# speedinghzl/DSRG

Hardware: AMD Instinct MI355X
Metric: images/sec DSRG train step (VGG16 321x321, 21-class) (higher is better)
Workload: dtype bf16 backbone (fp32 master weights) + f32/f64 supervision path

## Files before the change

dsrg_amd/csrc/conv_igemm.hip:

```cpp
#include "common.h"
#include "igemm_plan.h"
#include <algorithm>
#include <cstring>
#include <vector>

namespace dsrg {
namespace {
typedef __attribute__((ext_vector_type(8))) __bf16 bf16x8;
typedef __attribute__((ext_vector_type(2))) __bf16 bf16x2;
typedef __attribute__((ext_vector_type(2))) float f32x2;
typedef __attribute__((ext_vector_type(16))) float f32x16;
typedef __attribute__((ext_vector_type(4))) float f32x4;
typedef __attribute__((address_space(3))) void lds_void;

constexpr int kOutRow = 128 * 2 + 16;
constexpr int kOutWave = 64 * kOutRow;
constexpr uint32_t kOob = 0x80000000u;
constexpr int kRowTab = 8 * kOutWave;
constexpr int kRowTabBytes = kBM * 4;

template <int BK, int NST> struct ICfg {
    static constexpr int ROW = BK * 2;
    static constexpr int CPR = ROW / 16;
    static constexpr int RPI = 1024 / ROW;
    static constexpr int IPW = 256 / RPI / 8;
    static constexpr int STAGE = (kBM + kBN) * ROW;
    static constexpr int KS = BK / 16;
    static constexpr int SPC = 64 / BK;
    static constexpr int AHEAD = NST - 1;
    static_assert(NST * STAGE <= kRowTab, "the row table sits behind the stages");
    static constexpr size_t LDS = (size_t)kRowTab + kRowTabBytes;
    __device__ static constexpr int swz(int r) { return BK == 64 ? (r >> 1) & 7 : (r >> 2) & 3; }
};

struct IgemmClass {
    uint32_t rect;
    int q0;
};
struct IgemmGroup {
    const uint16_t *x;
    const uint16_t *w;
    const float *bias;
    uint16_t *y;
    const uint16_t *mask;
    float *colsum;
    const uint16_t *res;
    int dil, ncls;
    IgemmClass cls[kMaxClasses];
};
struct IgemmArgs {
    IgemmGroup g[4];
    int ngroups, B, H, W, Cin, Cout, taps, relu, M, tiles_m, tiles_n, tiles_per_group;
    int stagger;
    uint32_t drop_thresh;
    float drop_scale;
    uint32_t seed_lo, seed_hi;
    float out_scale;
    int xcd_mix;
    int row_tiles, rows_per_tile, bands;
    int skip_taps;
    int xrow;
    int cpp;
    int out_f32;
    int cls_tiles;
};

__device__ __forceinline__ uint32_t fmix32(uint32_t h) {
    h ^= h >> 16; h *= 0x85EBCA6Bu; h ^= h >> 13; h *= 0xC2B2AE35u; h ^= h >> 16;
    return h;
}
__device__ __forceinline__ uint32_t dropout_bytes(uint32_t e4, uint32_t seed_lo, uint32_t seed_hi) {
    return fmix32(fmix32(e4 ^ seed_lo) + seed_hi);
}

__device__ __forceinline__ uint32_t pack2(float lo, float hi) {
    f32x2 v = {lo, hi};
    bf16x2 b = __builtin_convertvector(v, bf16x2);
    return *reinterpret_cast<uint32_t *>(&b);
}

template <int N> __device__ __forceinline__ void wait_vm_barrier() {
    asm volatile("s_waitcnt vmcnt(%0)\n\ts_barrier" ::"n"(N) : "memory");
}

constexpr int kAhead = 3;
struct IgemmFrag {
    uint32_t choff[2];
    __device__ __forceinline__ explicit IgemmFrag(int lane) {
        using C = ICfg<64, 2>;
        const int l15 = lane & 15, g4 = lane >> 4;
#pragma unroll
        for (int sl = 0; sl < 2; sl++) choff[sl] = (uint32_t)l15 * C::ROW + (uint32_t)(((sl * 4 + g4) ^ C::swz(l15)) << 4);
    }
};
template <class LateIssue>
__device__ __forceinline__ void igemm_mma_step(const unsigned char *P, const unsigned char *Wt, const IgemmFrag &fr, f32x4 (&acc)[8][4],
                                               const bool late, LateIssue &&late_issue) {
    using C = ICfg<64, 2>;
    constexpr int RING = kAhead + 1;
    bf16x8 bq[2][4], ar[RING];
    auto read_w = [&](int u) { return *reinterpret_cast<const bf16x8 *>(Wt + (u & 7) * (16 * C::ROW) + fr.choff[u >> 3]); };
#pragma unroll
    for (int j = 0; j < 4; j++) bq[0][j] = *reinterpret_cast<const bf16x8 *>(P + j * (16 * C::ROW) + fr.choff[0]);
#pragma unroll
    for (int u = 0; u < kAhead; u++) ar[u] = read_w(u);
#pragma unroll
    for (int u = 0; u < 16; u++) {
        if (u + kAhead < 16) ar[(u + kAhead) % RING] = read_w(u + kAhead);
        if (u < 4) bq[1][u] = *reinterpret_cast<const bf16x8 *>(P + u * (16 * C::ROW) + fr.choff[1]);
        __builtin_amdgcn_sched_barrier(0);
#pragma unroll
        for (int j = 0; j < 4; j++)
            acc[u & 7][j] = __builtin_amdgcn_mfma_f32_16x16x32_bf16(ar[u % RING], bq[u >> 3][j], acc[u & 7][j], 0, 0, 0);
        __builtin_amdgcn_sched_barrier(0);
        if (u == 3 && late) late_issue();
    }
}

__device__ __forceinline__ void conv_igemm_body(const IgemmArgs &a, const int bid, const int nblk) {
    using C = ICfg<64, 2>;
    extern __shared__ __attribute__((aligned(16))) unsigned char ig_lds[];
    const int tid = threadIdx.x, lane = tid & 63;
    const int wv = __builtin_amdgcn_readfirstlane(tid >> 6);
    const int l15 = lane & 15, g4 = lane >> 4;
    const int wn = wv >> 2, wm = wv & 3;

    int grp, tm, tn;
    if (a.xcd_mix) {
        const int id = bid, xcd = id & 7, k = id >> 3;
        const int cm = (a.tiles_m - xcd + 7) >> 3, per_group = cm * a.tiles_n;
        if (cm <= 0 || k >= per_group * a.ngroups) return;
        grp = k / per_group;
        const int r = k - grp * per_group, tml = r / a.tiles_n;
        tn = r - tml * a.tiles_n;
        tm = xcd + 8 * tml;
    } else {
        const int total = nblk, id = bid;
        const int q = total >> 3, r = total & 7, xcd = id & 7, k = id >> 3;
        int t = (xcd < r ? xcd * (q + 1) : r * (q + 1) + (xcd - r) * q) + k;
        grp = t / a.tiles_per_group;
        t -= grp * a.tiles_per_group;
        tm = t / a.tiles_n;
        tn = t - tm * a.tiles_n;
    }
    int m0 = tm * kBM, mvalid;
    if (a.row_tiles) {
        const int bimg = tm / a.bands, band = tm - bimg * a.bands, row0 = band * a.rows_per_tile;
        m0 = (bimg * a.H + row0) * a.W;
        mvalid = min(a.rows_per_tile, a.H - row0) * a.W;
    } else {
        mvalid = min(kBM, a.M - m0);
    }
    const int n0 = tn * kBN;
    const IgemmGroup &G = a.g[grp];
    const int taps = a.taps, Cin = a.Cin, W = a.W, H = a.H;
    const int ktot = taps * Cin;
    volatile int32_t *rowpix = reinterpret_cast<volatile int32_t *>(ig_lds + kRowTab);
    const bool cls = a.cls_tiles != 0;
    if (cls) {
        if (tid < kBM) {
            const int q = m0 + tid;
            int m = -1;
            if (q < a.M) {
                uint32_t rect = G.cls[0].rect;
                int q0 = G.cls[0].q0;
#pragma unroll
                for (int k = 1; k < kMaxClasses; k++)
                    if (k < G.ncls && q >= G.cls[k].q0) { rect = G.cls[k].rect; q0 = G.cls[k].q0; }
                const int cy0 = (int)(rect & 255u), ch = (int)((rect >> 8) & 255u), cx0 = (int)((rect >> 16) & 255u), cw = (int)(rect >> 24);
                const int qq = q - q0, area = ch * cw, b = qq / area, rem = qq - b * area, yy = rem / cw, xx = rem - yy * cw;
                m = (b * H + cy0 + yy) * W + cx0 + xx;
            }
            rowpix[tid] = m;
        }
        __syncthreads();
    }
    auto row_pixel = [&](int r) -> int { return cls ? rowpix[r] : (r < mvalid ? m0 + r : -1); };

    const int xrow = a.xrow;
    const rsrc_t rx = make_rsrc(G.x, (size_t)a.M * xrow);
    const rsrc_t rw = make_rsrc(G.w, (size_t)a.Cout * ktot * 2);

    uint32_t pbase[C::IPW], pvalid[C::IPW], wbase[C::IPW];
#pragma unroll
    for (int i = 0; i < C::IPW; i++) {
        const int r = wv * 32 + i * C::RPI + lane / C::CPR;
        const int c = (lane % C::CPR) ^ C::swz(r);
        const int m = row_pixel(r);
        const bool in = m >= 0;
        const int mm = in ? m : 0;
        const int hw = H * W;
        const int b = mm / hw, rem = mm - b * hw, y = rem / W, x = rem - y * W;
        uint32_t valid = 0;
        if (in) {
            if (taps == 9) {
#pragma unroll
                for (int tap = 0; tap < 9; tap++) {
                    const int yy = y + (tap / 3 - 1) * G.dil, xx = x + (tap % 3 - 1) * G.dil;
                    if (yy >= 0 && yy < H && xx >= 0 && xx < W) valid |= 1u << tap;
                }
            } else {
                valid = 1u;
            }
        }
        pbase[i] = (uint32_t)mm * (uint32_t)xrow + (uint32_t)c * 16u;
        pvalid[i] = valid;
        wbase[i] = (uint32_t)(n0 + r) * (uint32_t)(ktot * 2) + (uint32_t)c * 16u;
    }

    uint32_t tapmask = taps == 9 ? 0x1ffu : 1u;
    if (a.skip_taps && taps == 9 && G.dil >= 3) {
        uint32_t v = 0;
#pragma unroll
        for (int i = 0; i < C::IPW; i++) v |= pvalid[i];
#pragma unroll
        for (int o = 32; o; o >>= 1) v |= (uint32_t)__shfl_xor((int)v, o);
        volatile uint32_t *red = reinterpret_cast<volatile uint32_t *>(ig_lds);
        if (lane == 0) red[wv] = v;
        __syncthreads();
        v = 0;
#pragma unroll
        for (int k = 0; k < 8; k++) v |= red[k];
        __syncthreads();
        tapmask = (uint32_t)__builtin_amdgcn_readfirstlane((int)v);
    }
    unsigned long long taplist = 0;
    int nlive = 0;
#pragma unroll
    for (int tp = 0; tp < 9; tp++)
        if ((tapmask >> tp) & 1u) { taplist |= (unsigned long long)tp << (4 * nlive); nlive++; }
    const int nsteps = (Cin >> 6) * nlive * C::SPC;

    int it_cc = 0, it_tap = 0, it_h = 0;
    auto issue = [&](int stage, int) {
        const int tap = (int)((taplist >> (4 * it_tap)) & 15u);
        const int cc = it_cc, h = it_h;
        const uint32_t s_real = (uint32_t)((cc * taps + tap) * C::SPC + h);
        if (++it_h == C::SPC) { it_h = 0; if (++it_tap == nlive) { it_tap = 0; it_cc++; } }
        int dy = 0, dx = 0;
        if (taps == 9) { dy = tap / 3 - 1; dx = tap - (tap / 3) * 3 - 1; }
        const int xc = a.cpp ? (int)((0x610u >> (2 * (cc / a.cpp))) & 3u) * a.cpp + cc % a.cpp : cc;
        const int toff = (dy * G.dil * W + dx * G.dil) * xrow + xc * 128 + h * C::ROW;
        unsigned char *P = ig_lds + stage * C::STAGE + wv * (32 * C::ROW);
        unsigned char *Wt = P + kBM * C::ROW;
#pragma unroll
        for (int i = 0; i < C::IPW; i++) {
            const uint32_t vo = ((pvalid[i] >> tap) & 1u) ? pbase[i] + (uint32_t)toff : kOob;
            __builtin_amdgcn_raw_ptr_buffer_load_lds(rx, (lds_void *)(P + i * (C::RPI * C::ROW)), 16, vo, 0, 0, 0);
        }
#pragma unroll
        for (int i = 0; i < C::IPW; i++)
            __builtin_amdgcn_raw_ptr_buffer_load_lds(rw, (lds_void *)(Wt + i * (C::RPI * C::ROW)), 16, wbase[i], s_real * C::ROW, 0, 0);
    };

    f32x4 acc[8][4];
#pragma unroll
    for (int i = 0; i < 8; i++)
#pragma unroll
        for (int j = 0; j < 4; j++)
#pragma unroll
            for (int r = 0; r < 4; r++) acc[i][j][r] = 0.0f;

    const IgemmFrag fr(lane);
    const bool active = n0 + wn * 128 < a.Cout;
    const bool late = a.stagger && wv >= 4 && active;
    if (nsteps > 0) issue(0, 0);
    if (!active) {
        for (int s = 0; s < nsteps; s++) {
            wait_vm_barrier<0>();
            if (s + 1 < nsteps) issue((s & 1) ^ 1, s + 1);
        }
    } else {
        for (int s = 0; s < nsteps; s++) {
            const int stage = s & 1;
            wait_vm_barrier<0>();
            const bool more = s + 1 < nsteps;
            if (more && !late) issue(stage ^ 1, s + 1);
            igemm_mma_step(ig_lds + stage * C::STAGE + wm * (64 * C::ROW), ig_lds + stage * C::STAGE + kBM * C::ROW + wn * (128 * C::ROW), fr, acc,
                           more && late, [&]() { issue(stage ^ 1, s + 1); });
        }
    }
    __syncthreads();
    if (!active) return;

    unsigned char *O = ig_lds + wv * kOutWave;
    const int nw = n0 + wn * 128;
    if (a.out_f32) {
        float *y32 = reinterpret_cast<float *>(G.y);
        const float floor32 = a.relu ? 0.0f : -__builtin_inff();
#pragma unroll
        for (int j = 0; j < 4; j++) {
            const int m = row_pixel(wm * 64 + j * 16 + l15);
#pragma unroll
            for (int i = 0; i < 8; i++) {
                const int n = nw + i * 16 + g4 * 4;
                float4 b4 = make_float4(0.f, 0.f, 0.f, 0.f);
                if (G.bias) b4 = *reinterpret_cast<const float4 *>(G.bias + n);
                const float4 v = make_float4(fmaxf(acc[i][j][0] + b4.x, floor32), fmaxf(acc[i][j][1] + b4.y, floor32),
                                             fmaxf(acc[i][j][2] + b4.z, floor32), fmaxf(acc[i][j][3] + b4.w, floor32));
                if (m >= 0) *reinterpret_cast<float4 *>(y32 + (size_t)m * a.Cout + n) = v;
            }
        }
        return;
    }
    const rsrc_t rb = make_rsrc(G.bias, G.bias ? (size_t)a.Cout * 4 : 0);
    const float floor_ = (a.relu && !G.res) ? 0.0f : -__builtin_inff();
    const uint32_t seed_g = a.seed_lo + (uint32_t)grp * 0x9E3779B9u;
    float bias_r[8][4];
#pragma unroll
    for (int i = 0; i < 8; i++)
#pragma unroll
        for (int e = 0; e < 4; e++) bias_r[i][e] = ld_f32(rb, (uint32_t)(nw + i * 16 + g4 * 4 + e) * 4u);
#pragma unroll
    for (int i = 0; i < 8; i++) {
        const int nl = i * 16 + g4 * 4;
#pragma unroll
        for (int j = 0; j < 4; j++) {
            float v0 = acc[i][j][0] + bias_r[i][0], v1 = acc[i][j][1] + bias_r[i][1];
            float v2 = acc[i][j][2] + bias_r[i][2], v3 = acc[i][j][3] + bias_r[i][3];
            v0 = fmaxf(v0, floor_) * a.out_scale; v1 = fmaxf(v1, floor_) * a.out_scale;
            v2 = fmaxf(v2, floor_) * a.out_scale; v3 = fmaxf(v3, floor_) * a.out_scale;
            if (a.drop_thresh) {
                const uint32_t m = cls ? (uint32_t)rowpix[wm * 64 + j * 16 + l15] : (uint32_t)(m0 + wm * 64 + j * 16 + l15);
                const uint32_t h = dropout_bytes((m * (uint32_t)a.Cout + (uint32_t)(nw + nl)) >> 2, seed_g, a.seed_hi);
                v0 = (h & 0xffu) >= a.drop_thresh ? v0 * a.drop_scale : 0.0f;
                v1 = ((h >> 8) & 0xffu) >= a.drop_thresh ? v1 * a.drop_scale : 0.0f;
                v2 = ((h >> 16) & 0xffu) >= a.drop_thresh ? v2 * a.drop_scale : 0.0f;
                v3 = (h >> 24) >= a.drop_thresh ? v3 * a.drop_scale : 0.0f;
            }
            *reinterpret_cast<uint2 *>(O + (j * 16 + l15) * kOutRow + nl * 2) = make_uint2(pack2(v0, v1), pack2(v2, v3));
        }
    }
    const bool chv = nw + (lane & 15) * 8 < a.Cout;
    if (G.res) {
        const float floor2 = a.relu ? 0.0f : -__builtin_inff();
#pragma unroll
        for (int h = 0; h < 2; h++) {
            uint4 rs[8], mk8[8];
#pragma unroll
            for (int it = 0; it < 8; it++) {
                const int m = row_pixel(wm * 64 + (h * 8 + it) * 4 + (lane >> 4));
                const size_t at = (size_t)m * a.Cout + nw + (lane & 15) * 8;
                rs[it] = (m >= 0 && chv) ? *reinterpret_cast<const uint4 *>(G.res + at) : make_uint4(0, 0, 0, 0);
                mk8[it] = !G.mask ? make_uint4(0x3f803f80u, 0x3f803f80u, 0x3f803f80u, 0x3f803f80u)
                                  : ((m >= 0 && chv) ? *reinterpret_cast<const uint4 *>(G.mask + at) : make_uint4(0, 0, 0, 0));
            }
#pragma unroll
            for (int it = 0; it < 8; it++) {
                const int p = (h * 8 + it) * 4 + (lane >> 4), ch = lane & 15;
                const int m = row_pixel(wm * 64 + p);
                const uint4 v = *reinterpret_cast<const uint4 *>(O + p * kOutRow + ch * 16);
                uint32_t w4[4] = {v.x, v.y, v.z, v.w};
                const uint32_t r4[4] = {rs[it].x, rs[it].y, rs[it].z, rs[it].w};
                const uint32_t y4[4] = {mk8[it].x, mk8[it].y, mk8[it].z, mk8[it].w};
#pragma unroll
                for (int e = 0; e < 4; e++) {
                    const float lo = fmaxf(__uint_as_float(w4[e] << 16) + __uint_as_float(r4[e] << 16), floor2);
                    const float hi = fmaxf(__uint_as_float(w4[e] & 0xffff0000u) + __uint_as_float(r4[e] & 0xffff0000u), floor2);
                    const uint32_t klo = (int16_t)(y4[e] & 0xffffu) > 0 ? 0x0000ffffu : 0u;
                    const uint32_t khi = (int32_t)y4[e] >= 0x10000 ? 0xffff0000u : 0u;
                    w4[e] = pack2(lo, hi) & (klo | khi);
                }
                if (m >= 0 && chv) *reinterpret_cast<uint4 *>(G.y + (size_t)m * a.Cout + nw + ch * 8) = make_uint4(w4[0], w4[1], w4[2], w4[3]);
            }
        }
        return;
    }
    if (!G.mask && !G.colsum) {
#pragma unroll 4
        for (int it = 0; it < 16; it++) {
            const int p = it * 4 + (lane >> 4), ch = lane & 15;
            const int m = row_pixel(wm * 64 + p);
            const uint4 v = *reinterpret_cast<const uint4 *>(O + p * kOutRow + ch * 16);
            if (m >= 0 && chv) *reinterpret_cast<uint4 *>(G.y + (size_t)m * a.Cout + nw + ch * 8) = v;
        }
        return;
    }
    uint4 mk[16];
    if (G.mask) {
#pragma unroll
        for (int it = 0; it < 16; it++) {
            const int m = row_pixel(wm * 64 + it * 4 + (lane >> 4));
            mk[it] = (m >= 0 && chv) ? *reinterpret_cast<const uint4 *>(G.mask + (size_t)m * a.Cout + nw + (lane & 15) * 8) : make_uint4(0, 0, 0, 0);
        }
    } else {
#pragma unroll
        for (int it = 0; it < 16; it++) mk[it] = make_uint4(0x3f803f80u, 0x3f803f80u, 0x3f803f80u, 0x3f803f80u);
    }
    float cs[8] = {0, 0, 0, 0, 0, 0, 0, 0};
#pragma unroll
    for (int it = 0; it < 16; it++) {
        const int p = it * 4 + (lane >> 4), ch = lane & 15;
        const int m = row_pixel(wm * 64 + p);
        const uint4 v = *reinterpret_cast<const uint4 *>(O + p * kOutRow + ch * 16);
        uint32_t w4[4] = {v.x, v.y, v.z, v.w};
        const uint32_t y4[4] = {mk[it].x, mk[it].y, mk[it].z, mk[it].w};
#pragma unroll
        for (int e = 0; e < 4; e++) {
            const uint32_t lo = (int16_t)(y4[e] & 0xffffu) > 0 ? 0x0000ffffu : 0u;
            const uint32_t hi = (int32_t)y4[e] >= 0x10000 ? 0xffff0000u : 0u;
            w4[e] &= lo | hi;
            cs[2 * e] += __uint_as_float(w4[e] << 16);
            cs[2 * e + 1] += __uint_as_float(w4[e] & 0xffff0000u);
        }
        if (m >= 0 && chv) *reinterpret_cast<uint4 *>(G.y + (size_t)m * a.Cout + nw + ch * 8) = make_uint4(w4[0], w4[1], w4[2], w4[3]);
    }
    if (G.colsum) {
#pragma unroll
        for (int e = 0; e < 8; e++) {
            cs[e] += __shfl_xor(cs[e], 16);
            cs[e] += __shfl_xor(cs[e], 32);
        }
        float *slab = reinterpret_cast<float *>(O);
        if (lane < 16) {
            *reinterpret_cast<float4 *>(slab + lane * 8) = make_float4(cs[0], cs[1], cs[2], cs[3]);
            *reinterpret_cast<float4 *>(slab + lane * 8 + 4) = make_float4(cs[4], cs[5], cs[6], cs[7]);
        }
        __syncthreads();
        if (wm == 0) {
            const float *s0 = reinterpret_cast<const float *>(ig_lds + (wn * 4 + 0) * kOutWave);
            const float *s1 = reinterpret_cast<const float *>(ig_lds + (wn * 4 + 1) * kOutWave);
            const float *s2 = reinterpret_cast<const float *>(ig_lds + (wn * 4 + 2) * kOutWave);
            const float *s3 = reinterpret_cast<const float *>(ig_lds + (wn * 4 + 3) * kOutWave);
            float *dst = G.colsum + (size_t)tm * a.Cout + nw;
            dst[lane] = (s0[lane] + s1[lane]) + (s2[lane] + s3[lane]);
            if (nw + lane + 64 < a.Cout) dst[lane + 64] = (s0[lane + 64] + s1[lane + 64]) + (s2[lane + 64] + s3[lane + 64]);
        }
    }
}


__global__ __launch_bounds__(512, 2) void conv_igemm_kernel_64x2(IgemmArgs a) { conv_igemm_body(a, (int)blockIdx.x, (int)gridDim.x); }

struct IgemmSkArgs {
    IgemmArgs base;
    float *ws;
    uint32_t *flags;
    int units, tiles_total;
};
constexpr int kSkParts = 4;
using f32x4v = decltype(__builtin_amdgcn_raw_buffer_load_b128(rsrc_t(), 0, 0, 0));

__global__ __launch_bounds__(512, 2) void conv_igemm_sk_kernel(IgemmSkArgs k) {
    using C = ICfg<64, 2>;
    const IgemmArgs &a = k.base;
    extern __shared__ __attribute__((aligned(16))) unsigned char ig_lds[];
    const int tid = threadIdx.x, lane = tid & 63;
    const int wv = __builtin_amdgcn_readfirstlane(tid >> 6);
    const int l15 = lane & 15, g4 = lane >> 4;
    const int wn = wv >> 2, wm = wv & 3;
    int unit;
    {
        const int total = (int)gridDim.x, id = (int)blockIdx.x;
        const int q = total >> 3, r = total & 7, xcd = id & 7, kk = id >> 3;
        unit = (xcd < r ? xcd * (q + 1) : r * (q + 1) + (xcd - r) * q) + kk;
    }
    const int taps = a.taps, Cin = a.Cin, W = a.W, H = a.H;
    const int ktot = taps * Cin;
    const int nsteps = (Cin >> 6) * taps;
    const long long total_steps = (long long)k.tiles_total * nsteps;
    auto unit_start = [&](int u) { return (long long)u * total_steps / k.units; };
    const long long g1 = unit_start(unit + 1);
    const IgemmFrag fr(lane);
    const rsrc_t rws = make_rsrc(k.ws, (size_t)k.units * 32 * 512 * 16);
    const float floor_ = a.relu ? 0.0f : -__builtin_inff();

    for (long long g = unit_start(unit); g < g1;) {
        const int tile = (int)(g / nsteps);
        const int sb = (int)(g - (long long)tile * nsteps);
        const int se = (int)min((long long)nsteps, sb + (g1 - g));
        int t = tile;
        const int grp = t / a.tiles_per_group;
        t -= grp * a.tiles_per_group;
        const int tm = t / a.tiles_n, tn = t - tm * a.tiles_n;
        const int m0 = tm * kBM, n0 = tn * kBN;
        const IgemmGroup G = a.g[grp];
        const rsrc_t rx = make_rsrc(G.x, (size_t)a.M * Cin * 2);
        const rsrc_t rw = make_rsrc(G.w, (size_t)a.Cout * ktot * 2);
        const bool active = n0 + wn * 128 < a.Cout;

        uint32_t pbase0, wbase0, pvalid01 = 0, pvalid23 = 0;
        {
            const int r0 = wv * 32 + lane / C::CPR;
            const int c0 = (lane % C::CPR) ^ C::swz(r0);
            pbase0 = (uint32_t)(m0 + r0) * (uint32_t)(Cin * 2) + (uint32_t)c0 * 16u;
            wbase0 = (uint32_t)(n0 + r0) * (uint32_t)(ktot * 2) + (uint32_t)c0 * 16u;
#pragma unroll
            for (int i = 0; i < C::IPW; i++) {
                const int m = m0 + r0 + i * C::RPI;
                uint32_t valid = 0;
                if (m < a.M) {
                    const int hw = H * W;
                    const int bimg = m / hw, rem = m - bimg * hw, y = rem / W, x = rem - y * W;
                    if (taps == 9) {
#pragma unroll
                        for (int tap = 0; tap < 9; tap++) {
                            const int yy = y + (tap / 3 - 1) * G.dil, xx = x + (tap % 3 - 1) * G.dil;
                            if (yy >= 0 && yy < H && xx >= 0 && xx < W) valid |= 1u << tap;
                        }
                    } else {
                        valid = 1u;
                    }
                }
                if (i < 2) pvalid01 |= valid << (16 * i); else pvalid23 |= valid << (16 * (i - 2));
            }
        }
        auto issue = [&](int stage, int s) {
            const int cc = s / taps, tap = s - cc * taps;
            int dy = 0, dx = 0;
            if (taps == 9) { dy = tap / 3 - 1; dx = tap - (tap / 3) * 3 - 1; }
            const int toff = (dy * G.dil * W + dx * G.dil) * Cin * 2 + cc * 128;
            unsigned char *P = ig_lds + stage * C::STAGE + wv * (32 * C::ROW);
            unsigned char *Wt = P + kBM * C::ROW;
#pragma unroll
            for (int i = 0; i < C::IPW; i++) {
                const uint32_t bits = (i < 2 ? pvalid01 : pvalid23) >> (16 * (i & 1) + tap);
                const uint32_t off = ((pbase0 + (uint32_t)(i * C::RPI * Cin * 2)) ^ ((i & 1) ? 64u : 0u)) + (uint32_t)toff;
                __builtin_amdgcn_raw_ptr_buffer_load_lds(rx, (lds_void *)(P + i * (C::RPI * C::ROW)), 16, (bits & 1u) ? off : kOob, 0, 0, 0);
            }
#pragma unroll
            for (int i = 0; i < C::IPW; i++)
                __builtin_amdgcn_raw_ptr_buffer_load_lds(rw, (lds_void *)(Wt + i * (C::RPI * C::ROW)), 16, (i & 1) ? wbase0 ^ 64u : wbase0,
                                                         (uint32_t)s * C::ROW + (uint32_t)(i * C::RPI * ktot * 2), 0, 0);
        };

        f32x4 acc[8][4];
#pragma unroll
        for (int i = 0; i < 8; i++)
#pragma unroll
            for (int j = 0; j < 4; j++)
#pragma unroll
                for (int r = 0; r < 4; r++) acc[i][j][r] = 0.0f;

        issue(0, sb);
        if (!active) {
            for (int s = sb; s < se; s++) {
                wait_vm_barrier<0>();
                if (s + 1 < se) issue(((s - sb) & 1) ^ 1, s + 1);
            }
        } else {
            for (int s = sb; s < se; s++) {
                const int stage = (s - sb) & 1;
                wait_vm_barrier<0>();
                const bool more = s + 1 < se, late = wv >= 4;
                if (more && !late) issue(stage ^ 1, s + 1);
                igemm_mma_step(ig_lds + stage * C::STAGE + wm * (64 * C::ROW), ig_lds + stage * C::STAGE + kBM * C::ROW + wn * (128 * C::ROW), fr, acc,
                               more && late, [&]() { issue(stage ^ 1, s + 1); });
            }
        }
        __syncthreads();

        if (sb != 0) {
            if (active) {
#pragma unroll
                for (int i = 0; i < 8; i++)
#pragma unroll
                    for (int j = 0; j < 4; j++) {
                        f32x4v v = {__float_as_uint(acc[i][j][0]), __float_as_uint(acc[i][j][1]), __float_as_uint(acc[i][j][2]), __float_as_uint(acc[i][j][3])};
                        __builtin_amdgcn_raw_buffer_store_b128(v, rws, (uint32_t)((i * 4 + j) * 512 + tid) * 16u,
                                                               (uint32_t)unit * (32u * 512u * 16u), 16);
                    }
            }
            asm volatile("s_waitcnt vmcnt(0)" ::: "memory");
            __syncthreads();
            if (tid == 0) __hip_atomic_store(k.flags + unit, 1u, __ATOMIC_RELAXED, __HIP_MEMORY_SCOPE_AGENT);
        } else {
            bool ok = true;
            int nparts = 0;
            if (se != nsteps) {
                const long long tile_end = (long long)(tile + 1) * nsteps;
                while (unit + 1 + nparts < k.units && unit_start(unit + 1 + nparts) < tile_end) nparts++;
                volatile int &sk_ok = *reinterpret_cast<volatile int *>(ig_lds);
                if (tid == 0) {
                    int good = nparts <= kSkParts ? 1 : 0;
                    for (int p = 0; p < nparts && good; p++) {
                        unsigned spins = 0;
                        while (__hip_atomic_load(k.flags + unit + 1 + p, __ATOMIC_RELAXED, __HIP_MEMORY_SCOPE_AGENT) != 1u) {
                            __builtin_amdgcn_s_sleep(8);
                            if (++spins > (1u << 24)) { good = 0; break; }
                        }
                    }
                    if (good) __builtin_amdgcn_fence(__ATOMIC_ACQUIRE, "agent");
                    else __hip_atomic_store(k.flags + k.units, 1u, __ATOMIC_RELAXED, __HIP_MEMORY_SCOPE_AGENT);
                    sk_ok = good;
                }
                __syncthreads();
                ok = sk_ok != 0;
                __syncthreads();
            }
            if (active) {
                const float poison = ok ? 0.0f : __builtin_nanf("");
                unsigned char *O = ig_lds + wv * kOutWave;
                const int nw = n0 + wn * 128;
                const rsrc_t rb = make_rsrc(G.bias, G.bias ? (size_t)a.Cout * 4 : 0);
                const uint32_t seed_g = a.seed_lo + (uint32_t)grp * 0x9E3779B9u;
                f32x4v shares[2][kSkParts];
                float bq[2][4];
                auto fetch = [&](int gi, f32x4v (&dst)[kSkParts], float (&bias4)[4]) {
                    const int i = gi >> 2;
                    const uint32_t off = (uint32_t)(gi * 512 + tid) * 16u;
#pragma unroll
                    for (int p = 0; p < kSkParts; p++)
                        dst[p] = __builtin_amdgcn_raw_buffer_load_b128(rws, p < nparts ? off : kOob, (uint32_t)(unit + 1 + p) * (32u * 512u * 16u), 0);
#pragma unroll
                    for (int e = 0; e < 4; e++) bias4[e] = ld_f32(rb, (uint32_t)(nw + i * 16 + g4 * 4 + e) * 4u);
                };
                fetch(0, shares[0], bq[0]);
#pragma unroll
                for (int gi = 0; gi < 32; gi++) {
                    const int i = gi >> 2, j = gi & 3;
                    if (gi + 1 < 32) fetch(gi + 1, shares[(gi + 1) & 1], bq[(gi + 1) & 1]);
                    __builtin_amdgcn_sched_barrier(0);
                    const int nl = i * 16 + g4 * 4;
                    float s0 = acc[i][j][0], s1 = acc[i][j][1], s2 = acc[i][j][2], s3 = acc[i][j][3];
#pragma unroll
                    for (int p = 0; p < kSkParts; p++) {
                        const f32x4v pv = shares[gi & 1][p];
                        s0 += __uint_as_float(pv[0]); s1 += __uint_as_float(pv[1]); s2 += __uint_as_float(pv[2]); s3 += __uint_as_float(pv[3]);
                    }
                    float v0 = s0 + bq[gi & 1][0], v1 = s1 + bq[gi & 1][1], v2 = s2 + bq[gi & 1][2], v3 = s3 + bq[gi & 1][3];
                    v0 = fmaxf(v0, floor_) + poison; v1 = fmaxf(v1, floor_) + poison; v2 = fmaxf(v2, floor_) + poison; v3 = fmaxf(v3, floor_) + poison;
                    if (a.drop_thresh) {
                        const uint32_t m = (uint32_t)(m0 + wm * 64 + j * 16 + l15);
                        const uint32_t h = dropout_bytes((m * (uint32_t)a.Cout + (uint32_t)(nw + nl)) >> 2, seed_g, a.seed_hi);
                        v0 = (h & 0xffu) >= a.drop_thresh ? v0 * a.drop_scale : 0.0f;
                        v1 = ((h >> 8) & 0xffu) >= a.drop_thresh ? v1 * a.drop_scale : 0.0f;
                        v2 = ((h >> 16) & 0xffu) >= a.drop_thresh ? v2 * a.drop_scale : 0.0f;
                        v3 = (h >> 24) >= a.drop_thresh ? v3 * a.drop_scale : 0.0f;
                    }
                    *reinterpret_cast<uint2 *>(O + (j * 16 + l15) * kOutRow + nl * 2) = make_uint2(pack2(v0, v1), pack2(v2, v3));
                    __builtin_amdgcn_sched_barrier(0);
                }
#pragma unroll 4
                for (int it = 0; it < 16; it++) {
                    const int p = it * 4 + (lane >> 4), ch = lane & 15;
                    const int m = m0 + wm * 64 + p;
                    const uint4 v = *reinterpret_cast<const uint4 *>(O + p * kOutRow + ch * 16);
                    if (m < a.M) *reinterpret_cast<uint4 *>(G.y + (size_t)m * a.Cout + nw + ch * 8) = v;
                }
            }
        }
        g += se - sb;
        __syncthreads();
    }
}

struct WgradGroup {
    const uint16_t *x;
    const uint16_t *g;
    float *part;
    int dil, pad_;
};
struct IgemmWgradArgs {
    WgradGroup g[4];
    int ngroups, B, H, W, Cin, Cout, taps, M, tiles_n, tiles_c, ksplit, kchunk, tiles_per_group;
    int stagger;
    int compact;
    int xcd_mix;
    int skip_rows;
    int nent;
    const uint32_t *plan;
};
constexpr int kWRow = 512;
constexpr int kWTile = 64 * kWRow;
constexpr int kWStage = 2 * kWTile;
typedef __attribute__((__vector_size__(4 * sizeof(__bf16)))) __bf16 bf16x4v;
typedef __attribute__((address_space(3))) unsigned char lds_u8;

__device__ __forceinline__ bf16x8 tr_frag8(lds_u8 *p) {
    bf16x4v lo = __builtin_amdgcn_ds_read_tr16_b64_v4bf16(reinterpret_cast<__attribute__((address_space(3))) bf16x4v *>(p));
    bf16x4v hi = __builtin_amdgcn_ds_read_tr16_b64_v4bf16(reinterpret_cast<__attribute__((address_space(3))) bf16x4v *>(p + 4 * kWRow));
    return __builtin_shufflevector(lo, hi, 0, 1, 2, 3, 4, 5, 6, 7);
}

__device__ __forceinline__ void conv_igemm_wgrad_body(const IgemmWgradArgs &a, const int bid, const int nblk) {
    extern __shared__ __attribute__((aligned(16))) unsigned char ig_lds[];
    const int tid = threadIdx.x, lane = tid & 63;
    const int wv = __builtin_amdgcn_readfirstlane(tid >> 6);
    const int l31 = lane & 31, kgrp = lane >> 5, i16 = lane & 15, gq = lane >> 4;
    const int wn = wv >> 2, wm = wv & 3;

    const int tiles = a.tiles_n * a.tiles_c;
    int grp, split, t, ksp = a.ksplit;
    size_t plane = 0;
    if (a.plan) {
        const int ncb_ = (a.Cin + 255) >> 8, tpe = a.tiles_n * ncb_;
        const int xcd = bid & 7, k = bid >> 3, pos = k / tpe, te = k - pos * tpe, e = pos * 8 + xcd;
        if (e >= a.nent) return;
        const uint32_t w = a.plan[kPlanHdr + e];
        grp = (int)(w & 3u);
        const int ptap = (int)((w >> 2) & 15u), tn_ = te / ncb_;
        split = (int)((w >> 6) & 255u);
        ksp = (int)((w >> 14) & 255u);
        t = tn_ * a.tiles_c + ptap * ncb_ + (te - tn_ * ncb_);
        plane = (size_t)a.plan[2 * (grp * 9 + ptap) + 1] + (size_t)split;
    } else if (a.xcd_mix) {
        const int id = bid, xcd = id & 7, k = id >> 3;
        if (a.ksplit >= 8) {
            const int per_group = (a.ksplit >> 3) * tiles;
            grp = k / per_group;
            const int r = k - grp * per_group, sl = r / tiles;
            t = r - sl * tiles;
            split = xcd + 8 * sl;
        } else {
            const int xpc = 8 / a.ksplit, sub = xcd % xpc, per_group = tiles / xpc;
            split = xcd / xpc;
            grp = k / per_group;
            t = sub + xpc * (k - grp * per_group);
        }
    } else {
        const int total = nblk, id = bid;
        const int q = total >> 3, r = total & 7, xcd = id & 7, k = id >> 3;
        t = (xcd < r ? xcd * (q + 1) : r * (q + 1) + (xcd - r) * q) + k;
        grp = t / a.tiles_per_group;
        t -= grp * a.tiles_per_group;
        split = t / tiles;
        t -= split * tiles;
    }
    const int tn = t / a.tiles_c, tc = t - tn * a.tiles_c;
    const WgradGroup G = a.g[grp];
    const int taps = a.taps, Cin = a.Cin, Cout = a.Cout, W = a.W, H = a.H;
    const bool two = Cin == 128 && taps == 9;
    const int ncb = two ? 1 : (Cin + 255) >> 8;
    const int tap = two ? 2 * tc : tc / ncb, c0 = two ? 0 : (tc - tap * ncb) << 8, n0 = tn << 8;
    const int tdy = (taps == 9 && !two) ? (tap / 3 - 1) * G.dil : 0, tdx = (taps == 9 && !two) ? (tap % 3 - 1) * G.dil : 0;
    const bool compact = a.compact && !two && taps == 9;
    const int ry0 = compact ? max(0, -tdy) : 0, rx0 = compact ? max(0, -tdx) : 0;
    const int rh_ = compact ? H - abs(tdy) : H, rw_ = compact ? W - abs(tdx) : W;
    const int rh = max(rh_, 1), rw = max(rw_, 1);
    const int area = rh * rw;
    const int Kc = (rh_ > 0 && rw_ > 0) ? a.B * area : 0;
    const int kchunk = compact ? (((Kc + ksp - 1) / ksp + 63) >> 6) << 6 : a.kchunk;
    const int mbeg = split * kchunk, mend = min(Kc, mbeg + kchunk);
    const int nsteps = mend > mbeg ? (mend - mbeg + 63) >> 6 : 0;

    const rsrc_t rx = make_rsrc(G.x, (size_t)a.M * Cin * 2);
    const rsrc_t rg = make_rsrc(G.g, (size_t)a.M * Cout * 2);

    int pm[4], pb[4], py[4], px[4], ldy[4], ldx[4], ltapoff[4];
    uint32_t srcoff[4], xsrcoff[4];
    bool ltap[4];
#pragma unroll
    for (int i = 0; i < 4; i++) {
        const int r = wv * 8 + i * 2 + (lane >> 5);
        const int q = lane & 31, p = (q >> 2) ^ (r & 3);
        srcoff[i] = (uint32_t)(p * 64 + (q & 3) * 16);
        const int mytap = two ? tap + (p >> 2) : tap;
        xsrcoff[i] = two ? (uint32_t)((p & 3) * 64 + (q & 3) * 16) : srcoff[i];
        if (!two && (uint32_t)(c0 * 2) + xsrcoff[i] >= (uint32_t)(Cin * 2)) xsrcoff[i] |= 0x80000000u;
        if ((uint32_t)(n0 * 2) + srcoff[i] >= (uint32_t)(Cout * 2)) srcoff[i] |= 0x80000000u;
        ltap[i] = mytap < taps;
        ldy[i] = taps == 9 ? (mytap / 3 - 1) * G.dil : 0;
        ldx[i] = taps == 9 ? (mytap % 3 - 1) * G.dil : 0;
        ltapoff[i] = (ldy[i] * W + ldx[i]) * Cin * 2 + c0 * 2;
        const int m = mbeg + r;
        pm[i] = m;
        const int mm = m < Kc ? m : 0;
        pb[i] = mm / area;
        const int rem = mm - pb[i] * area;
        py[i] = rem / rw;
        px[i] = rem - py[i] * rw;
    }
    const int qW = 64 / rw, rW = 64 - qW * rw;

    auto advance = [&]() {
#pragma unroll
        for (int i = 0; i < 4; i++) {
            pm[i] += 64;
            px[i] += rW;
            py[i] += qW;
            if (px[i] >= rw) { px[i] -= rw; py[i] += 1; }
            while (py[i] >= rh) { py[i] -= rh; pb[i] += 1; }
        }
    };
    auto issue = [&](int stage) {
        unsigned char *A = ig_lds + stage * kWStage + wv * (8 * kWRow);
        unsigned char *Bt = A + kWTile;
        int pix[4];
#pragma unroll
        for (int i = 0; i < 4; i++) pix[i] = compact ? (pb[i] * H + ry0 + py[i]) * W + rx0 + px[i] : pm[i];
#pragma unroll
        for (int i = 0; i < 4; i++) {
            const bool live = pm[i] < mend;
            const uint32_t vo = live ? (uint32_t)pix[i] * (uint32_t)(Cout * 2) + (uint32_t)(n0 * 2) + srcoff[i] : kOob;
            __builtin_amdgcn_raw_ptr_buffer_load_lds(rg, (lds_void *)(A + i * (2 * kWRow)), 16, vo, 0, 0, 0);
        }
#pragma unroll
        for (int i = 0; i < 4; i++) {
            const int yy = ry0 + py[i] + ldy[i], xx = rx0 + px[i] + ldx[i];
            const bool live = ltap[i] && pm[i] < mend && yy >= 0 && yy < H && xx >= 0 && xx < W;
            const uint32_t vo = live ? (uint32_t)(pix[i] * (Cin * 2) + ltapoff[i]) + xsrcoff[i] : kOob;
            __builtin_amdgcn_raw_ptr_buffer_load_lds(rx, (lds_void *)(Bt + i * (2 * kWRow)), 16, vo, 0, 0, 0);
        }
        advance();
    };

    f32x16 acc[4][2];
#pragma unroll
    for (int i = 0; i < 4; i++)
#pragma unroll
        for (int j = 0; j < 2; j++)
#pragma unroll
            for (int r = 0; r < 16; r++) acc[i][j][r] = 0.0f;

    const int swz = (i16 >> 2) & 3;
    const uint32_t lane_off = (uint32_t)((kgrp * 8 + (i16 >> 2)) * kWRow + (gq & 1) * 32 + (i16 & 3) * 8);
    uint32_t aoff[4], boff[2];
#pragma unroll
    for (int i = 0; i < 4; i++) aoff[i] = lane_off + (uint32_t)(((wn * 4 + i) ^ swz) * 64);
#pragma unroll
    for (int j = 0; j < 2; j++) boff[j] = lane_off + (uint32_t)(kWTile + ((wm * 2 + j) ^ swz) * 64);
    lds_u8 *lds = (lds_u8 *)ig_lds;

    const bool may_skip = a.skip_rows && !compact && abs(tdy) * W >= 64 && tdy > -H && tdy < H;
    const int hw_ = H * W;
    auto step_dead = [&](int st) -> bool {
        const int p0 = mbeg + st * 64, p1 = min(p0 + 63, mend - 1);
        const int b0 = p0 / hw_, b1 = p1 / hw_;
        if (b0 != b1) return false;
        const int y0 = (p0 - b0 * hw_) / W, y1 = (p1 - b0 * hw_) / W;
        return y1 + tdy < 0 || y0 + tdy >= H;
    };
    int cur = 0;
    auto seek = [&]() {
        if (may_skip)
            while (cur < nsteps && step_dead(cur)) { advance(); cur++; }
    };
    seek();
    bool have = cur < nsteps;
    if (have) { issue(0); cur++; }
    for (int s = 0; have; s++) {
        wait_vm_barrier<0>();
        seek();
        const bool more = cur < nsteps, late = a.stagger && wv >= 4;
        if (more && !late) { issue((s + 1) & 1); cur++; }
        lds_u8 *st = lds + (s & 1) * kWStage;
        bf16x8 af[2][4], bfr[2][2];
#pragma unroll
        for (int i = 0; i < 4; i++) af[0][i] = tr_frag8(st + aoff[i]);
#pragma unroll
        for (int j = 0; j < 2; j++) bfr[0][j] = tr_frag8(st + boff[j]);
#pragma unroll
        for (int ks = 0; ks < 4; ks++) {
            if (ks + 1 < 4) {
#pragma unroll
                for (int i = 0; i < 4; i++) af[(ks + 1) & 1][i] = tr_frag8(st + (ks + 1) * (16 * kWRow) + aoff[i]);
#pragma unroll
                for (int j = 0; j < 2; j++) bfr[(ks + 1) & 1][j] = tr_frag8(st + (ks + 1) * (16 * kWRow) + boff[j]);
            }
            __builtin_amdgcn_sched_barrier(0);
#pragma unroll
            for (int i = 0; i < 4; i++)
#pragma unroll
                for (int j = 0; j < 2; j++)
                    acc[i][j] = __builtin_amdgcn_mfma_f32_32x32x16_bf16(af[ks & 1][i], bfr[ks & 1][j], acc[i][j], 0, 0, 0);
            __builtin_amdgcn_sched_barrier(0);
            if (ks == 0 && more && late) { issue((s + 1) & 1); cur++; }
        }
        have = more;
    }
    float *pp = a.plan ? G.part + plane * ((size_t)Cout * Cin) : G.part + (size_t)split * ((size_t)Cout * taps * Cin);
    const size_t prow = a.plan ? (size_t)Cin : (size_t)taps * Cin;
#pragma unroll
    for (int i = 0; i < 4; i++)
#pragma unroll
        for (int j = 0; j < 2; j++) {
            const int col = wm * 64 + j * 32 + l31;
            const int etap = two ? tap + (col >> 7) : tap, c = two ? (col & 127) : c0 + col;
            if (etap < taps && c < Cin && n0 + wn * 128 + i * 32 < Cout) {
#pragma unroll
                for (int r = 0; r < 16; r++) {
                    const int n = n0 + wn * 128 + i * 32 + (r & 3) + 8 * (r >> 2) + 4 * kgrp;
                    pp[(size_t)n * prow + (a.plan ? 0 : etap * Cin) + c] = acc[i][j][r];
                }
            }
        }
}

__global__ __launch_bounds__(512, 2) void conv_igemm_wgrad_kernel(IgemmWgradArgs a) { conv_igemm_wgrad_body(a, (int)blockIdx.x, (int)gridDim.x); }

struct IgemmBwdArgs {
    IgemmArgs d;
    IgemmWgradArgs w;
    int nd, nd_pad, nw;
    int w_first, nw_pad;
};
__global__ __launch_bounds__(512, 2) void conv_igemm_bwd_kernel(IgemmBwdArgs a) {
    const int id = (int)blockIdx.x;
    if (a.w_first) {
        if (id < a.nw_pad) {
            if (id < a.nw) conv_igemm_wgrad_body(a.w, id, a.nw);
        } else if (id - a.nw_pad < a.nd) {
            conv_igemm_body(a.d, id - a.nw_pad, a.nd);
        }
        return;
    }
    if (id < a.nd_pad) {
        if (id < a.nd) conv_igemm_body(a.d, id, a.nd);
    } else {
        conv_igemm_wgrad_body(a.w, id - a.nd_pad, a.nw);
    }
}

struct WgradReduceArgs {
    const float *part[4];
    void *gw[4];
    int ksplit;
    int cin4;
    const uint32_t *plan;
    size_t plane4;
    size_t n4;
    const float *scale;
    size_t per_o4;
};
template <bool BF16_OUT>
__global__ __launch_bounds__(256) void conv_igemm_wgrad_reduce_kernel(WgradReduceArgs a) {
    const size_t e = (size_t)blockIdx.x * 256 + threadIdx.x;
    if (e >= a.n4) return;
    const float4 *p = reinterpret_cast<const float4 *>(a.part[blockIdx.y]) + e;
    void *gw = a.gw[blockIdx.y];
    int ksplit = a.ksplit;
    size_t stride = a.n4;
    if (a.plan) {
        const size_t n = e / a.per_o4, rem = e - n * a.per_o4;
        const int tap = (int)(rem / (size_t)a.cin4), c4 = (int)(rem - (size_t)tap * a.cin4);
        const uint32_t *row = a.plan + 2 * ((int)blockIdx.y * 9 + tap);
        ksplit = (int)row[0];
        stride = a.plane4;
        p = reinterpret_cast<const float4 *>(a.part[0]) + (size_t)row[1] * a.plane4 + n * (size_t)a.cin4 + c4;
    }
    float4 s = ksplit > 0 ? p[0] : make_float4(0.0f, 0.0f, 0.0f, 0.0f);
    int k = 1;
    for (; k + 8 <= ksplit; k += 8) {
        float4 v[8];
#pragma unroll
        for (int u = 0; u < 8; u++) v[u] = p[(size_t)(k + u) * stride];
#pragma unroll
        for (int u = 0; u < 8; u++) { s.x += v[u].x; s.y += v[u].y; s.z += v[u].z; s.w += v[u].w; }
    }
    for (; k < ksplit; k++) {
        const float4 v = p[(size_t)k * stride];
        s.x += v.x; s.y += v.y; s.z += v.z; s.w += v.w;
    }
    if (a.scale) {
        const float f = a.scale[e / a.per_o4];
        s.x *= f; s.y *= f; s.z *= f; s.w *= f;
    }
    if (BF16_OUT) reinterpret_cast<uint2 *>(gw)[e] = make_uint2(pack2(s.x, s.y), pack2(s.z, s.w));
    else reinterpret_cast<float4 *>(gw)[e] = s;
}


__global__ __launch_bounds__(256) void pack_conv_weight_kernel(const float *w, uint16_t *fwd, uint16_t *dg, int cout, int cin, int taps,
                                                               int plain, const float *scale) {
    __shared__ uint16_t tile[64][64 + 4];
    const int ob = blockIdx.x, cb = blockIdx.y, tap = blockIdx.z, t = threadIdx.x;
    const int r = t >> 4, q = t & 15;
#pragma unroll
    for (int i = 0; i < 4; i++) {
        const int o = r + 16 * i;
        const size_t src = ((size_t)(ob * 64 + o) * taps + tap) * cin + cb * 64 + q * 4;
        float4 v = *reinterpret_cast<const float4 *>(w + src);
        if (scale) {
            const float f = scale[ob * 64 + o];
            v.x *= f; v.y *= f; v.z *= f; v.w *= f;
        }
        const uint2 pk = make_uint2(pack2(v.x, v.y), pack2(v.z, v.w));
        if (fwd) *reinterpret_cast<uint2 *>(fwd + (plain ? src : (((size_t)(ob * 64 + o) * (cin >> 6) + cb) * taps + tap) * 64 + q * 4)) = pk;
        *reinterpret_cast<uint2 *>(&tile[o][q * 4]) = pk;
    }
    if (!dg) return;
    __syncthreads();
#pragma unroll
    for (int i = 0; i < 4; i++) {
        const int c = r + 16 * i;
        const uint32_t lo = (uint32_t)tile[q * 4 + 0][c] | ((uint32_t)tile[q * 4 + 1][c] << 16);
        const uint32_t hi = (uint32_t)tile[q * 4 + 2][c] | ((uint32_t)tile[q * 4 + 3][c] << 16);
        const size_t dst = plain ? ((size_t)(cb * 64 + c) * taps + (taps - 1 - tap)) * cout + ob * 64 + q * 4
                                 : (((size_t)(cb * 64 + c) * (cout >> 6) + ob) * taps + (taps - 1 - tap)) * 64 + q * 4;
        *reinterpret_cast<uint2 *>(dg + dst) = make_uint2(lo, hi);
    }
}

}

bool conv_igemm_supported(int cin, int cout, int k) {
    return (k == 1 || k == 3) && cin >= 64 && cin % 64 == 0 && cout >= 128 && cout % 128 == 0;
}

std::atomic<int> g_igemm_variant{-1};
static IgemmVariant igemm_variant() { return decode_igemm_variant(g_igemm_variant.load(std::memory_order_relaxed)); }

static int igemm_cus() {
    static const int n = [] {
        int dev = 0, c = 0;
        if (hipGetDevice(&dev) != hipSuccess || hipDeviceGetAttribute(&c, hipDeviceAttributeMultiprocessorCount, dev) != hipSuccess || c < 8) c = 256;
        return c;
    }();
    return n;
}
size_t conv_igemm_workspace() { return (size_t)igemm_cus() * (32 * 512 * 16) + ((size_t)igemm_cus() + 1 + 63) / 64 * 256; }

struct ColsumArgs {
    const float *part[4];
    float *out[4];
    int rows, cout;
};
__global__ __launch_bounds__(1024) void igemm_colsum_kernel(ColsumArgs a) {
    __shared__ float red[16][64];
    colsum_block(a.part[blockIdx.y], a.out[blockIdx.y], a.rows, a.cout, (int)blockIdx.x, red);
}

int launch_igemm_colsum(const float *const *parts, float *const *outs, int ngroups, int rows, int cout, hipStream_t stream) {
    if (ngroups < 1 || ngroups > 4 || cout % 64 || rows < 1) return set_error(DSRG_ERR_INVALID, "column sums: 1..4 groups, 64 | channels");
    if (defer_reduction(0, ngroups, parts, outs, rows, cout)) return DSRG_OK;
    ColsumArgs c;
    memset(&c, 0, sizeof(c));
    for (int g = 0; g < ngroups; g++) { c.part[g] = parts[g]; c.out[g] = outs[g]; }
    c.rows = rows; c.cout = cout;
    hipLaunchKernelGGL(igemm_colsum_kernel, dim3(cout / 64, ngroups), dim3(1024), 0, stream, c);
    DSRG_LAUNCH_CHECK();
    return DSRG_OK;
}

size_t conv_igemm_colsum_workspace(int ngroups, int B, int H, int W, int cout) {
    return (size_t)ngroups * conv_igemm_pixel_tiles(B, H, W) * (size_t)cout * sizeof(float);
}

namespace {
struct IgemmLaunch {
    IgemmSkArgs sk;
    int grid;
    bool stream_k;
};

int prepare_igemm(const IgemmRequest &r, const IgemmVariant &v, IgemmLaunch &L) {
    const int ngroups = r.ngroups, B = r.s.B, H = r.s.H, W = r.s.W, cin = r.s.cin, cout = r.s.cout, k = r.s.k, split_cin = r.split_cin;
    const float drop_p = r.drop_p;
    if (ngroups < 1 || ngroups > 4) return set_error(DSRG_ERR_INVALID, "conv_igemm: 1..4 groups");
    if (r.colsums && (!r.colsum_ws || r.colsum_ws_bytes < conv_igemm_colsum_workspace(ngroups, B, H, W, cout)))
        return set_error(DSRG_ERR_INVALID, "conv_igemm: column-sum scratch missing or too small");
    if (!conv_igemm_launchable(cin, cout, k))
        return set_error(DSRG_ERR_UNSUPPORTED, "conv_igemm: cin %% 64 == 0, cout %% 128 == 0 (or cout = 64), k in (1, 3) required (got %d, %d, %d)",
                         cin, cout, k);
    const long long M = (long long)B * H * W;
    if (M <= 0 || M * cin * 2 >= 0x7fffffffLL || (long long)cout * k * k * cin * 2 >= 0x7fffffffLL || M * cout * 2 >= 0x7fffffff00LL)
        return set_error(DSRG_ERR_UNSUPPORTED, "conv_igemm: tensor too large for 32-bit buffer offsets");
    memset(&L, 0, sizeof(L));
    IgemmArgs &a = L.sk.base;
    for (int g = 0; g < ngroups; g++) {
        a.g[g].x = static_cast<const uint16_t *>(r.x[g]);
        a.g[g].w = static_cast<const uint16_t *>(r.w[g]);
        a.g[g].bias = r.bias[g];
        a.g[g].y = static_cast<uint16_t *>(r.y[g]);
        a.g[g].dil = r.dil[g];
        a.g[g].mask = r.masked ? static_cast<const uint16_t *>(r.mask[g]) : nullptr;
        a.g[g].colsum = r.colsums ? static_cast<float *>(r.colsum_ws) + (size_t)g * conv_igemm_pixel_tiles(B, H, W) * cout : nullptr;
        a.g[g].res = static_cast<const uint16_t *>(r.res);
        if (!a.g[g].x || !a.g[g].w || !a.g[g].y || (r.masked && !r.mask[g]) || (r.colsums && !r.colsum[g]))
            return set_error(DSRG_ERR_INVALID, "conv_igemm: null pointer");
    }
    a.out_scale = r.out_scale;
    a.xrow = cin * 2;
    if (split_cin > 0) {
        a.xrow = 3 * split_cin * 2;
        a.cpp = split_cin / 64;
        a.out_f32 = 1;
    }
    a.skip_taps = v.skip_dead_steps;
    const bool fused_bwd = r.masked || r.colsums || r.res;
    if (r.res && (r.colsums || ngroups != 1 || drop_p != 0.0f || split_cin))
        return set_error(DSRG_ERR_UNSUPPORTED, "conv_igemm: a residual goes with one group, no column sums, no dropout");
    a.ngroups = ngroups; a.B = B; a.H = H; a.W = W; a.Cin = cin; a.Cout = cout; a.taps = k * k; a.relu = r.relu; a.M = (int)M;
    a.tiles_m = (int)((M + kBM - 1) / kBM);
    a.tiles_n = (cout + kBN - 1) / kBN;
    a.tiles_per_group = a.tiles_m * a.tiles_n;
    if (drop_p < 0.0f || drop_p >= 1.0f) return set_error(DSRG_ERR_INVALID, "conv_igemm: 0 <= dropout probability < 1");
    a.drop_thresh = (uint32_t)(drop_p * 256.0f + 0.5f);
    if (a.drop_thresh > 255) a.drop_thresh = 255;
    a.drop_scale = 256.0f / (float)(256 - (int)a.drop_thresh);
    a.seed_lo = (uint32_t)r.seed; a.seed_hi = (uint32_t)(r.seed >> 32);
    a.stagger = v.stagger;
    const int units = igemm_cus(), tiles_total = a.tiles_per_group * ngroups, nsteps = (cin / 64) * k * k;
    const bool sk_wins = tiles_total * 100 <= units * 60;
    if (r.may_stream_k && !fused_bwd && split_cin == 0 && cout % 128 == 0 && r.workspace && r.workspace_bytes >= conv_igemm_workspace() &&
        ((v.stream_k_where_it_wins && sk_wins) || v.stream_k_forced) && (long long)tiles_total * nsteps >= (long long)units * 8 &&
        tiles_total * 3 >= units) {
        L.stream_k = true; L.grid = units;
        a.stagger = 1;
        L.sk.ws = static_cast<float *>(r.workspace);
        L.sk.flags = reinterpret_cast<uint32_t *>(static_cast<unsigned char *>(r.workspace) + (size_t)units * (32 * 512 * 16));
        L.sk.units = units; L.sk.tiles_total = tiles_total;
        return DSRG_OK;
    }
    int dils[4];
    for (int g = 0; g < ngroups; g++) {
        dils[g] = a.g[g].dil;
        if (a.skip_taps && k == 3 && dils[g] >= 3) a.xcd_mix = 1;
    }
    const bool rows_ok = a.xcd_mix && W <= kBM && conv_igemm_row_tiles(H, W);
    if (a.xcd_mix && v.class_tiles_allowed && H <= 255 && W <= 255 && (class_order_pays(B, H, W, dils, ngroups, rows_ok) || v.class_tiles_forced)) {
        a.cls_tiles = 1;
        for (int g = 0; g < ngroups; g++) {
            HostClass c[kMaxClasses];
            const int n = build_classes(H, W, dils[g], c);
            long long q0 = 0;
            a.g[g].ncls = n;
            for (int i = 0; i < n; i++) {
                a.g[g].cls[i].rect = (uint32_t)c[i].y0 | (uint32_t)(c[i].y1 - c[i].y0) << 8 | (uint32_t)c[i].x0 << 16 | (uint32_t)(c[i].x1 - c[i].x0) << 24;
                a.g[g].cls[i].q0 = (int)q0;
                q0 += (long long)B * (c[i].y1 - c[i].y0) * (c[i].x1 - c[i].x0);
            }
        }
    }
    if (!a.cls_tiles && rows_ok) {
        a.row_tiles = 1;
        a.rows_per_tile = kBM / W;
        a.bands = (H + a.rows_per_tile - 1) / a.rows_per_tile;
        a.tiles_m = B * a.bands;
        a.tiles_per_group = a.tiles_m * a.tiles_n;
    }
    L.grid = a.xcd_mix ? 8 * ngroups * ((a.tiles_m + 7) / 8) * a.tiles_n : a.tiles_per_group * ngroups;
    return DSRG_OK;
}

int run_colsum(const IgemmArgs &a, float *const *colsum, hipStream_t stream) {
    if (!colsum) return DSRG_OK;
    const float *parts[4];
    for (int g = 0; g < a.ngroups; g++) parts[g] = a.g[g].colsum;
    return launch_igemm_colsum(parts, colsum, a.ngroups, a.tiles_m, a.Cout, stream);
}

int run_igemm(const IgemmLaunch &L, float *const *colsum, hipStream_t stream) {
    static LdsGrant grant[2];
    constexpr size_t lds = ICfg<64, 2>::LDS;
    const IgemmArgs &a = L.sk.base;
    if (L.stream_k) {
        if (int rc = ensure_dynamic_lds(reinterpret_cast<const void *>(&conv_igemm_sk_kernel), lds, grant[1])) return rc;
        DSRG_HIP_CHECK(hipMemsetAsync(L.sk.flags, 0, sizeof(uint32_t) * ((size_t)L.sk.units + 1), stream));
        hipLaunchKernelGGL(conv_igemm_sk_kernel, dim3(L.grid), dim3(512), lds, stream, L.sk);
        DSRG_LAUNCH_CHECK();
        return DSRG_OK;
    }
    if (int rc = ensure_dynamic_lds(reinterpret_cast<const void *>(&conv_igemm_kernel_64x2), lds, grant[0])) return rc;
    hipLaunchKernelGGL(conv_igemm_kernel_64x2, dim3(L.grid), dim3(512), lds, stream, a);
    DSRG_LAUNCH_CHECK();
    return run_colsum(a, colsum, stream);
}
}

int launch_conv_igemm(const IgemmRequest &r, hipStream_t stream) {
    IgemmLaunch L;
    if (int rc = prepare_igemm(r, igemm_variant(), L)) return rc;
    return run_igemm(L, r.colsums ? r.colsum : nullptr, stream);
}

int launch_conv_igemm_split(const void *x3, const void *w, const float *bias, float *y, int dil, const ConvGeom &s, int relu, hipStream_t stream) {
    if (!conv_igemm_supported(s.cin, s.cout, s.k) || (long long)s.B * s.H * s.W * 3 * s.cin * 2 >= 0x7fffffffLL)
        return set_error(DSRG_ERR_UNSUPPORTED, "conv_igemm_split: shape not supported");
    IgemmRequest r;
    r.x[0] = x3; r.w[0] = w; r.bias[0] = bias; r.y[0] = y; r.dil[0] = dil;
    r.s = {s.B, s.H, s.W, 6 * s.cin, s.cout, s.k};
    r.relu = relu;
    r.split_cin = s.cin;
    return launch_conv_igemm(r, stream);
}

bool conv_igemm_wgrad_supported(int cin, int cout, int k) {
    return (k == 1 || k == 3) && ((cin >= 256 && cin % 256 == 0) || (cin == 128 && k == 3)) && cout >= 256 && cout % 256 == 0;
}

size_t conv_igemm_wgrad_workspace(int ngroups, int B, int H, int W, int cin, int cout, int k) {
    return wgrad_workspace_bytes(ngroups, B, H, W, cin, cout, k);
}

int conv_igemm_wgrad_splits(int ngroups, int B, int H, int W, int cin, int cout, int k, const int *dil, int *splits) {
    if (ngroups < 1 || ngroups > 4 || !splits || !conv_igemm_wgrad_launchable(cin, cout, k) || (long long)B * H * W <= 0)
        return set_error(DSRG_ERR_INVALID, "conv_igemm_wgrad_splits: 1..4 groups of a geometry conv_igemm_wgrad takes");
    if (wgrad_wants_plan(igemm_variant(), dil, ngroups, cin, k)) {
        const WgradPlan &p = build_wgrad_plan(ngroups, B, H, W, cin, cout, dil, igemm_cus());
        for (int i = 0; i < ngroups * 9; i++) splits[i] = (int)p.words[2 * i];
        return DSRG_OK;
    }
    const int ks = wgrad_uniform_ksplit(ngroups, (long long)B * H * W, cin, cout, k, wgrad_wants_mix(dil, ngroups, k));
    for (int i = 0; i < ngroups * k * k; i++) splits[i] = ks;
    return DSRG_OK;
}

constexpr int kPlanChunk = 960;
struct PlanChunkArgs { uint32_t *dst; int n, pad_; uint32_t w[kPlanChunk]; };
__global__ void __launch_bounds__(256) conv_igemm_wgrad_plan_kernel(const PlanChunkArgs c) {
    for (int i = threadIdx.x; i < c.n; i += 256) c.dst[i] = c.w[i];
}

namespace {
struct WgradLaunch {
    IgemmWgradArgs a;
    const WgradPlan *plan;
    int grid;
};

int prepare_wgrad(const WgradRequest &r, const IgemmVariant &v, WgradLaunch &L) {
    const int ngroups = r.ngroups, B = r.s.B, H = r.s.H, W = r.s.W, cin = r.s.cin, cout = r.s.cout, k = r.s.k, forced_ksplit = r.forced_ksplit;
    const int *const dil = r.dil;
    void *const workspace = r.workspace;
    if (ngroups < 1 || ngroups > 4) return set_error(DSRG_ERR_INVALID, "conv_igemm_wgrad: 1..4 groups");
    if (!conv_igemm_wgrad_launchable(cin, cout, k))
        return set_error(DSRG_ERR_UNSUPPORTED, "conv_igemm_wgrad: cin %% 64 == 0, cout %% 64 == 0, k in (1, 3) required (got %d, %d, %d)", cin, cout, k);
    const long long M = (long long)B * H * W;
    if (M <= 0 || M * cin * 2 >= 0x7fffffffLL || M * cout * 2 >= 0x7fffffffLL)
        return set_error(DSRG_ERR_UNSUPPORTED, "conv_igemm_wgrad: tensor too large for 32-bit buffer offsets");
    const size_t need = wgrad_workspace_bytes(ngroups, B, H, W, cin, cout, k);
    if (!workspace || r.workspace_bytes < need) return set_error(DSRG_ERR_INVALID, "conv_igemm_wgrad: workspace of %zu bytes needed", need);
    memset(&L, 0, sizeof(L));
    IgemmWgradArgs &a = L.a;
    a.ngroups = ngroups; a.B = B; a.H = H; a.W = W; a.Cin = cin; a.Cout = cout; a.taps = k * k; a.M = (int)M;
    a.tiles_n = (cout + 255) / 256;
    a.tiles_c = wgrad_col_tiles(cin, k);
    if (forced_ksplit <= 0 && wgrad_wants_plan(v, dil, ngroups, cin, k)) L.plan = &build_wgrad_plan(ngroups, B, H, W, cin, cout, dil, igemm_cus());
    a.ksplit = forced_ksplit > 0 ? forced_ksplit : wgrad_uniform_ksplit(ngroups, M, cin, cout, k, wgrad_wants_mix(dil, ngroups, k));
    a.kchunk = (int)(((M + a.ksplit - 1) / a.ksplit + 63) / 64 * 64);
    a.tiles_per_group = a.tiles_n * a.tiles_c * a.ksplit;
    a.stagger = v.stagger;
    a.skip_rows = v.skip_dead_steps;
    const size_t per_group = (size_t)a.ksplit * cout * k * k * cin;
    for (int q = 0; q < ngroups; q++) {
        a.g[q].x = static_cast<const uint16_t *>(r.x[q]);
        a.g[q].g = static_cast<const uint16_t *>(r.g[q]);
        a.g[q].part = static_cast<float *>(workspace) + (L.plan ? 0 : (size_t)q * per_group);
        a.g[q].dil = dil[q];
        if (!a.g[q].x || !a.g[q].g || !r.gw[q]) return set_error(DSRG_ERR_INVALID, "conv_igemm_wgrad: null pointer");
    }
    for (int q = 0; q < ngroups; q++) {
        if (a.skip_rows && k == 3 && a.g[q].dil >= 3 &&
            (a.ksplit % 8 == 0 || (8 % a.ksplit == 0 && (a.tiles_n * a.tiles_c) % (8 / a.ksplit) == 0))) a.xcd_mix = 1;
        if (a.skip_rows && v.wgrad_compact && k == 3 && cin != 128 && a.g[q].dil >= 1) a.compact = 1;
    }
    L.grid = a.tiles_per_group * ngroups;
    if (L.plan) {
        const size_t room = wgrad_plan_room(ngroups, wgrad_ksplit_bound(ngroups, B, H, W, cin, cout, k), cin, k);
        if (L.plan->words.size() * sizeof(uint32_t) > room || (size_t)L.plan->planes * cout * cin * sizeof(float) > need - room)
            return set_error(DSRG_ERR_INVALID, "conv_igemm_wgrad: work list larger than its workspace");
        a.plan = reinterpret_cast<uint32_t *>(static_cast<char *>(workspace) + (need - room));
        a.nent = L.plan->nent;
        L.grid = (a.nent + 7) / 8 * 8 * (a.tiles_n * ((cin + 255) / 256));
    }
    return DSRG_OK;
}

int upload_wgrad_plan(const WgradLaunch &L, hipStream_t stream) {
    if (!L.plan) return DSRG_OK;
    for (size_t at = 0, n = L.plan->words.size(); at < n; at += kPlanChunk) {
        PlanChunkArgs c;
        c.dst = const_cast<uint32_t *>(L.a.plan) + at;
        c.n = (int)std::min<size_t>(kPlanChunk, n - at);
        c.pad_ = 0;
        memcpy(c.w, L.plan->words.data() + at, (size_t)c.n * sizeof(uint32_t));
        hipLaunchKernelGGL(conv_igemm_wgrad_plan_kernel, dim3(1), dim3(256), 0, stream, c);
        DSRG_LAUNCH_CHECK();
    }
    return DSRG_OK;
}

int launch_wgrad(const WgradLaunch &L, hipStream_t stream) {
    static LdsGrant grant;
    constexpr size_t lds = 2 * kWStage;
    if (int rc = ensure_dynamic_lds(reinterpret_cast<const void *>(&conv_igemm_wgrad_kernel), lds, grant)) return rc;
    hipLaunchKernelGGL(conv_igemm_wgrad_kernel, dim3((unsigned)L.grid), dim3(512), lds, stream, L.a);
    DSRG_LAUNCH_CHECK();
    return DSRG_OK;
}

int reduce_wgrad(const IgemmWgradArgs &a, void *const *gw, const float *scale, int out_bf16, hipStream_t stream) {
    WgradReduceArgs r;
    memset(&r, 0, sizeof(r));
    r.ksplit = a.ksplit;
    r.plan = a.plan;
    r.cin4 = a.Cin / 4;
    r.plane4 = (size_t)a.Cout * a.Cin / 4;
    r.n4 = (size_t)a.Cout * a.taps * a.Cin / 4;
    r.scale = scale;
    r.per_o4 = (size_t)a.taps * a.Cin / 4;
    for (int q = 0; q < a.ngroups; q++) { r.part[q] = a.g[q].part; r.gw[q] = gw[q]; }
    const dim3 rgrid((unsigned)((r.n4 + 255) / 256), (unsigned)a.ngroups);
    if (out_bf16) hipLaunchKernelGGL(conv_igemm_wgrad_reduce_kernel<true>, rgrid, dim3(256), 0, stream, r);
    else hipLaunchKernelGGL(conv_igemm_wgrad_reduce_kernel<false>, rgrid, dim3(256), 0, stream, r);
    DSRG_LAUNCH_CHECK();
    return DSRG_OK;
}

int run_wgrad(const WgradLaunch &L, void *const *gw, const float *scale, int out_bf16, hipStream_t stream) {
    if (int rc = upload_wgrad_plan(L, stream)) return rc;
    if (int rc = launch_wgrad(L, stream)) return rc;
    return reduce_wgrad(L.a, gw, scale, out_bf16, stream);
}
}

int launch_conv_igemm_wgrad(const WgradRequest &r, int out_bf16, hipStream_t stream) {
    WgradLaunch L;
    if (int rc = prepare_wgrad(r, igemm_variant(), L)) return rc;
    return run_wgrad(L, r.gw, nullptr, out_bf16, stream);
}

static int launch_bwd_grid(const IgemmBwdArgs &a, hipStream_t stream) {
    static LdsGrant grant;
    constexpr size_t lds = ICfg<64, 2>::LDS > (size_t)(2 * kWStage) ? ICfg<64, 2>::LDS : (size_t)(2 * kWStage);
    if (int rc = ensure_dynamic_lds(reinterpret_cast<const void *>(&conv_igemm_bwd_kernel), lds, grant)) return rc;
    hipLaunchKernelGGL(conv_igemm_bwd_kernel, dim3(a.w_first ? a.nw_pad + a.nd : a.nd_pad + a.nw), dim3(512), lds, stream, a);
    DSRG_LAUNCH_CHECK();
    return DSRG_OK;
}

namespace {
struct Backward {
    IgemmLaunch d;
    WgradLaunch w;
    bool merge;
    int w_first;
};

IgemmRequest dgrad_half(const BackwardRequest &r) {
    IgemmRequest q;
    put_groups(q.x, r.g, 4); put_groups(q.w, r.wd, 4); put_groups(q.y, r.gx, 4); put_groups(q.mask, r.mask, 4);
    put_groups(q.colsum, r.bias_grad, 4); put_groups(q.dil, r.dil, 4);
    q.masked = r.masked; q.colsums = r.bias_grads; q.ngroups = r.ngroups;
    q.s = {r.s.B, r.s.H, r.s.W, r.s.cout, r.s.cin, r.s.k};
    q.out_scale = r.mask_scale;
    q.colsum_ws = r.colsum_ws; q.colsum_ws_bytes = r.colsum_ws_bytes;
    q.res = r.res;
    q.may_stream_k = false;
    return q;
}
WgradRequest wgrad_half(const BackwardRequest &r, int forced_ksplit) {
    WgradRequest q;
    put_groups(q.x, r.x, 4); put_groups(q.g, r.g, 4); put_groups(q.gw, r.gw, 4); put_groups(q.dil, r.dil, 4);
    q.ngroups = r.ngroups;
    q.workspace = r.wgrad_ws; q.workspace_bytes = r.wgrad_ws_bytes;
    q.s = r.s;
    q.forced_ksplit = forced_ksplit;
    return q;
}

int prepare_backward(const BackwardRequest &r, const IgemmVariant &v, Backward &P) {
    if (int rc = prepare_igemm(dgrad_half(r), v, P.d)) return rc;
    const int dil = r.dil[0], k = r.s.k;
    const bool merge = ((k == 3 && dil < 3) || k == 1) && v.merged_backward && !P.d.sk.base.xcd_mix && P.d.grid >= 1;
    const std::pair<int, int> pick = merge ? merged_backward_split(r.s.B, r.s.H, r.s.W, r.s.cin, r.s.cout, k, P.d.grid, igemm_cus()) : std::make_pair(0, 0);
    if (int rc = prepare_wgrad(wgrad_half(r, pick.first), v, P.w)) return rc;
    P.merge = merge && P.w.grid >= 1;
    P.w_first = pick.second;
    return DSRG_OK;
}

int prepare_backward_groups(const BackwardRequest &r, const IgemmVariant &v, Backward &P, MergedGroupsPlan &plan) {
    const int ngroups = r.ngroups, B = r.s.B, H = r.s.H, W = r.s.W, cin = r.s.cin, cout = r.s.cout, k = r.s.k;
    if (int rc = prepare_igemm(dgrad_half(r), v, P.d)) return rc;
    if (int rc = prepare_wgrad(wgrad_half(r, 0), v, P.w)) return rc;
    const IgemmArgs &a = P.d.sk.base;
    const DgradShape ds = dgrad_shape_for(ngroups, B, H, W, cin, cout, k, r.dil, v);
    const WgradShape ws = wgrad_shape_for(ngroups, B, H, W, cin, cout, k, r.dil, v, 0, igemm_cus());
    if (ds.grid != P.d.grid || ds.tiles_m != a.tiles_m || ds.tiles_n != a.tiles_n || ds.xcd_mix != a.xcd_mix || ds.row_tiles != a.row_tiles ||
        ds.cls_tiles != a.cls_tiles || ws.grid != P.w.grid || ws.ksplit != P.w.a.ksplit || ws.xcd_mix != P.w.a.xcd_mix ||
        ws.compact != P.w.a.compact || ws.nent != P.w.a.nent || (ws.plan != nullptr) != (P.w.plan != nullptr))
        return set_error(DSRG_ERR_INVALID, "conv_igemm_backward_groups: the planner and the launcher disagree on the grid");
    plan = MergedGroupsPlan{false, 0, P.w.plan ? 0 : P.w.a.ksplit, 0.0, 0.0};
    if (v.merged_backward && P.d.grid >= 1 && P.w.grid >= 1) {
        plan = merged_groups_plan(ds, cin, cout, k, v, P.w.plan ? 0 : r.forced_ksplit, igemm_cus());
        if (plan.merge && r.forced_order > 0) plan.w_first = r.forced_order == 2;
        if (plan.ksplit > 0 && plan.ksplit != P.w.a.ksplit)
            if (int rc = prepare_wgrad(wgrad_half(r, plan.ksplit), v, P.w)) return rc;
    }
    P.merge = plan.merge;
    P.w_first = plan.w_first;
    return DSRG_OK;
}

int run_backward(const Backward &P, void *const *gw, const float *gw_scale, float *const *bias_grad, hipStream_t stream) {
    if (!P.merge) {
        if (int rc = run_igemm(P.d, bias_grad, stream)) return rc;
        return run_wgrad(P.w, gw, gw_scale, 0, stream);
    }
    if (int rc = upload_wgrad_plan(P.w, stream)) return rc;
    IgemmBwdArgs a;
    memset(&a, 0, sizeof(a));
    a.d = P.d.sk.base;
    a.w = P.w.a;
    a.nd = P.d.grid; a.nd_pad = merged_second_half_start(a.nd); a.nw = P.w.grid; a.nw_pad = merged_second_half_start(a.nw);
    a.w_first = P.w_first;
    if (int rc = launch_bwd_grid(a, stream)) return rc;
    if (int rc = run_colsum(a.d, bias_grad, stream)) return rc;
    return reduce_wgrad(a.w, gw, gw_scale, 0, stream);
}
}

int launch_conv_igemm_backward(const BackwardRequest &r, hipStream_t stream) {
    Backward P;
    if (int rc = prepare_backward(r, igemm_variant(), P)) return rc;
    return run_backward(P, r.gw, r.gw_scale, r.bias_grads ? r.bias_grad : nullptr, stream);
}

int launch_conv_igemm_backward_groups(const BackwardRequest &r, hipStream_t stream) {
    if (r.bias_grads && !r.masked) return set_error(DSRG_ERR_INVALID, "conv_igemm_backward_groups: bias gradients come with the masks");
    Backward P;
    MergedGroupsPlan plan;
    if (int rc = prepare_backward_groups(r, igemm_variant(), P, plan)) return rc;
    return run_backward(P, r.gw, nullptr, r.bias_grads ? r.bias_grad : nullptr, stream);
}

int conv_igemm_backward_groups_plan(int ngroups, const ConvGeom &s, const int *dil, int with_mask, int forced_ksplit, int forced_order, int *out,
                                    double *us) {
    if (ngroups < 1 || ngroups > 4 || !out || !us) return set_error(DSRG_ERR_INVALID, "conv_igemm_backward_groups_plan: 1..4 groups");
    void *const fake = reinterpret_cast<void *>(uintptr_t(256));
    BackwardRequest r;
    for (int q = 0; q < ngroups; q++) {
        r.g[q] = r.wd[q] = r.x[q] = r.gx[q] = r.gw[q] = fake;
        if (with_mask) { r.mask[q] = fake; r.bias_grad[q] = static_cast<float *>(fake); }
    }
    r.masked = r.bias_grads = with_mask != 0;
    put_groups(r.dil, dil, ngroups);
    r.ngroups = ngroups;
    r.s = s;
    r.colsum_ws = with_mask ? fake : nullptr;
    r.colsum_ws_bytes = conv_igemm_colsum_workspace(ngroups, s.B, s.H, s.W, s.cin);
    r.wgrad_ws = fake;
    r.wgrad_ws_bytes = wgrad_workspace_bytes(ngroups, s.B, s.H, s.W, s.cin, s.cout, s.k);
    r.forced_ksplit = forced_ksplit; r.forced_order = forced_order;
    Backward P;
    MergedGroupsPlan plan;
    if (int rc = prepare_backward_groups(r, igemm_variant(), P, plan)) return rc;
    out[0] = plan.merge; out[1] = plan.w_first; out[2] = plan.ksplit; out[3] = P.d.grid; out[4] = P.w.grid;
    us[0] = plan.merged_us; us[1] = plan.separate_us;
    return DSRG_OK;
}

int launch_pack_conv_weight(const float *w, void *fwd, void *dgrad, int cout, int cin, int k, hipStream_t stream, int plain, const float *scale) {
    if (!w || cout < 64 || cout % 64 || cin < 64 || cin % 64 || (k != 1 && k != 3))
        return set_error(DSRG_ERR_INVALID, "pack_conv_weight: 64 | cout, 64 | cin, k in (1, 3) required (got %d, %d, %d)", cout, cin, k);
    if (!fwd && !dgrad) return DSRG_OK;
    hipLaunchKernelGGL(pack_conv_weight_kernel, dim3(cout / 64, cin / 64, k * k), dim3(256), 0, stream, w, static_cast<uint16_t *>(fwd),
                       static_cast<uint16_t *>(dgrad), cout, cin, k * k, plain, scale);
    DSRG_LAUNCH_CHECK();
    return DSRG_OK;
}

int conv_igemm_workspace_status(const void *workspace, hipStream_t stream, int *status) {
    uint32_t v = 0;
    const unsigned char *p = static_cast<const unsigned char *>(workspace) + (size_t)igemm_cus() * (32 * 512 * 16) + sizeof(uint32_t) * (size_t)igemm_cus();
    DSRG_HIP_CHECK(hipMemcpyAsync(&v, p, sizeof(v), hipMemcpyDeviceToHost, stream));
    DSRG_HIP_CHECK(hipStreamSynchronize(stream));
    *status = (int)v;
    return DSRG_OK;
}

}
```

dsrg_amd/csrc/igemm_plan.h:

```cpp
#pragma once
#include <algorithm>
#include <array>
#include <cstdint>
#include <cstdlib>
#include <functional>
#include <map>
#include <mutex>
#include <queue>
#include <vector>

namespace dsrg {

constexpr int kBM = 256, kBN = 256;
constexpr int kMaxClasses = 9;
constexpr int kPlanHdr = 2 * 4 * 9;

struct IgemmVariant {
    bool stagger;
    bool skip_dead_steps;
    bool stream_k_where_it_wins;
    bool stream_k_forced;
    bool class_tiles_allowed;
    bool class_tiles_forced;
    bool wgrad_work_list;
    bool wgrad_compact;
    bool merged_backward;
};
inline IgemmVariant decode_igemm_variant(int v) {
    const int e = (v < 0 || v == 2 || v == 5) ? 3 : v;
    return IgemmVariant{e >= 3, e != 6, e == 3 || e == 8 || e == 9, e == 4, e != 8, e == 9, e != 6 && e != 7, e != 7, e == 3 || e == 1 || e == 8 || e == 9};
}

template <class Key, class Value> struct PlanMemo {
    std::mutex mutex_;
    std::map<Key, Value> map_;
    template <class Make> const Value &get(const Key &key, Make &&make) {
        std::lock_guard<std::mutex> lock(mutex_);
        auto it = map_.find(key);
        if (it == map_.end()) it = map_.emplace(key, make()).first;
        return it->second;
    }
};

template <class Cost> double dispatch_makespan(int cus, Cost &&cost) {
    const int per_xcd = cus / 8 > 0 ? cus / 8 : 32;
    double worst = 0.0;
    for (int x = 0; x < 8; x++) {
        std::priority_queue<double, std::vector<double>, std::greater<double>> cu;
        for (int c = 0; c < per_xcd; c++) cu.push(0.0);
        double t;
        for (int b = 0; (t = cost(x, b)) >= 0.0; b++) {
            const double end = cu.top() + t;
            cu.pop();
            cu.push(end);
            worst = std::max(worst, end);
        }
    }
    return worst;
}

inline bool conv_igemm_launchable(int cin, int cout, int k) {
    return (k == 1 || k == 3) && cin >= 64 && cin % 64 == 0 && (cout == 64 || (cout >= 128 && cout % 128 == 0));
}
inline bool conv_igemm_wgrad_launchable(int cin, int cout, int k) {
    return (k == 1 || k == 3) && cin >= 64 && cin % 64 == 0 && cout >= 64 && cout % 64 == 0;
}
inline int wgrad_col_tiles(int cin, int k) { return (cin == 128 && k == 3) ? (k * k + 1) / 2 : k * k * ((cin + 255) / 256); }

inline bool conv_igemm_row_tiles(int H, int W) {
    if (W > kBM / 2) return false;
    const int r = kBM / W, bands = (H + r - 1) / r;
    return (long long)bands * kBM * 10 <= (long long)H * W * 11 + 10LL * kBM;
}
inline size_t conv_igemm_pixel_tiles(int B, int H, int W) {
    const long long M = (long long)B * H * W;
    size_t t = (size_t)((M + kBM - 1) / kBM);
    if (W <= kBM && conv_igemm_row_tiles(H, W)) {
        const int r = kBM / W;
        const size_t tr = (size_t)B * ((H + r - 1) / r);
        if (tr > t) t = tr;
    }
    return t;
}

inline uint32_t tap_mask_rect(int H, int W, int d, int y0, int y1, int x0, int x1) {
    uint32_t m = 0;
    for (int tap = 0; tap < 9; tap++) {
        const int dy = (tap / 3 - 1) * d, dx = (tap % 3 - 1) * d;
        if (std::max(y0, -dy) < std::min(y1, H - dy) && std::max(x0, -dx) < std::min(x1, W - dx)) m |= 1u << tap;
    }
    return m;
}
inline int axis_bands(int n, int d, int (*out)[2]) {
    if (d >= n) { out[0][0] = 0; out[0][1] = n; return 1; }
    const int lo = std::min(d, n - d), hi = std::max(d, n - d), cut[4] = {0, lo, hi, n};
    int k = 0;
    for (int i = 0; i < 3; i++)
        if (cut[i + 1] > cut[i]) { out[k][0] = cut[i]; out[k][1] = cut[i + 1]; k++; }
    return k;
}
struct HostClass { int y0, y1, x0, x1; uint32_t mask; };
inline int build_classes(int H, int W, int d, HostClass *c) {
    int yb[3][2], xb[3][2];
    const int ny = axis_bands(H, d, yb), nx = axis_bands(W, d, xb);
    int n = 0;
    for (int i = 0; i < ny; i++)
        for (int j = 0; j < nx; j++) c[n++] = HostClass{yb[i][0], yb[i][1], xb[j][0], xb[j][1], tap_mask_rect(H, W, d, yb[i][0], yb[i][1], xb[j][0], xb[j][1])};
    std::stable_sort(c, c + n, [](const HostClass &a, const HostClass &b) { return __builtin_popcount(a.mask) > __builtin_popcount(b.mask); });
    return n;
}
inline long long tile_taps(int B, int H, int W, int d, int mode) {
    const long long M = (long long)B * H * W;
    long long tot = 0;
    if (mode == 1) {
        const int r = kBM / W;
        for (int y0 = 0; y0 < H; y0 += r) tot += (long long)B * __builtin_popcount(tap_mask_rect(H, W, d, y0, std::min(H, y0 + r), 0, W));
        return tot;
    }
    HostClass c[kMaxClasses];
    const int n = mode == 2 ? build_classes(H, W, d, c) : 0;
    long long q0[kMaxClasses + 1] = {0};
    for (int k = 0; k < n; k++) q0[k + 1] = q0[k] + (long long)B * (c[k].y1 - c[k].y0) * (c[k].x1 - c[k].x0);
    for (long long t0 = 0; t0 < M; t0 += kBM) {
        const long long t1 = std::min(M, t0 + kBM);
        uint32_t m = 0;
        for (int k = 0; k < n; k++)
            if (q0[k] < t1 && q0[k + 1] > t0) m |= c[k].mask;
        for (long long p = t0; mode == 0 && p < t1;) {
            const int rem = (int)(p % ((long long)H * W)), y = rem / W, x = rem % W;
            const int x1 = (int)std::min<long long>(W, x + (t1 - p));
            m |= tap_mask_rect(H, W, d, y, y + 1, x, x1);
            p += x1 - x;
        }
        tot += __builtin_popcount(m);
    }
    return tot;
}
inline bool class_order_pays(int B, int H, int W, const int *dil, int ngroups, bool rows) {
    static PlanMemo<std::array<int, 9>, bool> memo;
    std::array<int, 9> key = {B, H, W, 0, 0, 0, 0, ngroups, rows};
    for (int g = 0; g < ngroups; g++) key[3 + g] = dil[g];
    return memo.get(key, [&] {
        long long now = 0, then = 0;
        for (int g = 0; g < ngroups; g++) { now += tile_taps(B, H, W, dil[g], 2); then += tile_taps(B, H, W, dil[g], rows ? 1 : 0); }
        return now * 100 < then * 97;
    });
}

inline int wgrad_ksplit(long long M, int tiles, int cus, double out_bytes = 0.0, bool xcd_mix_only = false) {
    long long best_cost = -1;
    int best = 1;
    for (int ks = 1; ks <= 128; ks++) {
        const long long chunk = ((M + ks - 1) / ks + 63) / 64 * 64;
        if ((long long)(ks - 1) * chunk >= M) continue;
        if (xcd_mix_only && ks % 8 != 0 && 8 % ks != 0) continue;
        const long long steps = chunk / 64, rounds = ((long long)tiles * ks + cus - 1) / cus;
        const long long cost = rounds * (steps + 8) + (long long)(ks * out_bytes / 9.2e6);
        if (best_cost < 0 || cost < best_cost) { best_cost = cost; best = ks; }
    }
    return best;
}
inline bool wgrad_wants_mix(const int *dil, int ngroups, int k) {
    for (int q = 0; q < ngroups; q++)
        if (k == 3 && dil && dil[q] >= 3) return true;
    return false;
}
inline int wgrad_uniform_ksplit(int ngroups, long long M, int cin, int cout, int k, bool xcd_mix_only) {
    return wgrad_ksplit(M, ngroups * ((cout + 255) / 256) * wgrad_col_tiles(cin, k), 256, (double)ngroups * cout * k * k * cin * 4.0, xcd_mix_only);
}

inline int wgrad_ksplit_cap(long long M, int ks) {
    const long long most = (M + 63) / 64;
    long long c = 2LL * ks;
    if (c > most) c = most;
    if (c > 128) c = 128;
    return (int)(c < ks ? ks : c);
}

inline int wgrad_ksplit_bound(int ngroups, int B, int H, int W, int cin, int cout, int k) {
    const long long M = (long long)B * H * W;
    int ks = std::max(wgrad_uniform_ksplit(ngroups, M, cin, cout, k, false), wgrad_uniform_ksplit(ngroups, M, cin, cout, k, true));
    if (ngroups == 1) ks = wgrad_ksplit_cap(M, ks);
    return ks;
}
inline size_t wgrad_plan_room(int ngroups, int ks_bound, int cin, int k) {
    if (k != 3 || cin == 128) return 0;
    return ((size_t)(kPlanHdr + ngroups * 9 * ks_bound) * sizeof(uint32_t) + 255) / 256 * 256;
}
inline size_t wgrad_workspace_bytes(int ngroups, int B, int H, int W, int cin, int cout, int k) {
    if (!conv_igemm_wgrad_launchable(cin, cout, k) || ngroups < 1 || ngroups > 4) return 0;
    const int ks = wgrad_ksplit_bound(ngroups, B, H, W, cin, cout, k);
    return (size_t)ngroups * ks * cout * k * k * cin * sizeof(float) + wgrad_plan_room(ngroups, ks, cin, k);
}

struct WgradPlan {
    std::vector<uint32_t> words;
    int nent = 0, planes = 0;
};
inline bool wgrad_wants_plan(const IgemmVariant &v, const int *dil, int ngroups, int cin, int k) {
    if (k != 3 || cin == 128 || !dil || !v.wgrad_work_list) return false;
    for (int q = 0; q < ngroups; q++)
        if (dil[q] < 1) return false;
    return wgrad_wants_mix(dil, ngroups, k);
}
inline const WgradPlan &build_wgrad_plan(int ngroups, int B, int H, int W, int cin, int cout, const int *dil, int cus) {
    static PlanMemo<std::array<int, 11>, WgradPlan> memo;
    std::array<int, 11> key = {B, H, W, cin, cout, ngroups, 0, 0, 0, 0, cus};
    for (int q = 0; q < ngroups; q++) key[6 + q] = dil[q];
    return memo.get(key, [&] {
        const int ntap = ngroups * 9, tpe = ((cout + 255) / 256) * ((cin + 255) / 256);
        const int cap = ntap * wgrad_ksplit_bound(ngroups, B, H, W, cin, cout, 3);
        const double plane_price = (double)cout * cin * 4.0 / 9.2e6;
        std::vector<long long> Kc(ntap);
        long long max_steps = 1;
        for (int q = 0; q < ngroups; q++)
            for (int tap = 0; tap < 9; tap++) {
                const int rh = H - abs((tap / 3 - 1) * dil[q]), rw = W - abs((tap % 3 - 1) * dil[q]);
                Kc[q * 9 + tap] = (rh > 0 && rw > 0) ? (long long)B * rh * rw : 0;
                max_steps = std::max(max_steps, (Kc[q * 9 + tap] + 63) / 64);
            }
        struct Entry { int steps, grp, tap, split, count; };
        auto chunk_of = [&](int i, long long c) { return ((Kc[i] + c - 1) / c + 63) / 64 * 64; };
        auto count_for = [&](int i, long long L) -> int {
            const long long steps = (Kc[i] + 63) / 64;
            long long c = std::min<long long>(std::max<long long>((steps + L / 2) / L, 1), 128);
            while (c > 1 && (c - 1) * chunk_of(i, c) >= Kc[i]) c--;
            return (int)c;
        };
        auto entries_for = [&](std::vector<Entry> &out, const int *cnt) {
            out.clear();
            for (int i = 0; i < ntap; i++)
                for (int s = 0; s < cnt[i]; s++) {
                    const long long ch = chunk_of(i, cnt[i]), beg = s * ch, end = std::min(Kc[i], beg + ch);
                    out.push_back({(int)((end - beg + 63) / 64), i / 9, i % 9, s, cnt[i]});
                }
            std::stable_sort(out.begin(), out.end(), [](const Entry &x, const Entry &y) { return x.steps > y.steps; });
        };
        auto makespan = [&](const std::vector<Entry> &es) {
            return dispatch_makespan(cus, [&](int x, int b) {
                const size_t e = (size_t)x + 8 * (size_t)(b / tpe);
                return e < es.size() ? (double)(es[e].steps + 8) : -1.0;
            });
        };
        std::vector<Entry> es, best_es;
        std::array<int, 36> counts{}, prev_counts{}, best_counts{};
        double best = -1.0;
        auto counts_for = [&](long long L) -> int {
            int planes = 0;
            for (int i = 0; i < ntap; i++) planes += (counts[i] = Kc[i] ? count_for(i, L) : 0);
            return planes;
        };
        for (long long L = max_steps; L >= 1; L--) {
            const int planes = counts_for(L);
            if (planes > cap) break;
            if (L < max_steps && counts == prev_counts) continue;
            prev_counts = counts;
            entries_for(es, counts.data());
            const double cost = makespan(es) + planes * plane_price;
            if (best < 0.0 || cost < best) { best = cost; best_es = es; best_counts = counts; }
        }
        WgradPlan p;
        p.words.assign(kPlanHdr, 0u);
        for (int i = 0, plane = 0; i < ntap; i++) {
            p.words[2 * i] = (uint32_t)best_counts[i];
            p.words[2 * i + 1] = (uint32_t)plane;
            plane += best_counts[i];
            p.planes = plane;
        }
        for (const Entry &e : best_es)
            p.words.push_back((uint32_t)e.grp | (uint32_t)e.tap << 2 | (uint32_t)e.split << 6 | (uint32_t)e.count << 14);
        p.nent = (int)best_es.size();
        return p;
    });
}

inline std::pair<int, int> merged_backward_split(int B, int H, int W, int cin, int cout, int k, int nd, int cus) {
    static PlanMemo<std::array<int, 8>, std::pair<int, int>> memo;
    return memo.get({B, H, W, cin, cout, k, nd, cus}, [&] {
        const long long M = (long long)B * H * W;
        const int tiles = ((cout + 255) / 256) * wgrad_col_tiles(cin, k), ks0 = wgrad_uniform_ksplit(1, M, cin, cout, k, false), cap = wgrad_ksplit_cap(M, ks0);
        const double td = ((cout / 64) * k * k + 6) * 1.85;
        auto makespan = [&](int n0, double t0, int n1, double t1) {
            return dispatch_makespan(cus, [&](int x, int b) {
                const int n0x = std::max((n0 - x + 7) / 8, 0), n1x = std::max((n1 - x + 7) / 8, 0);
                return b < n0x ? t0 : b < n0x + n1x ? t1 : -1.0;
            });
        };
        const bool order_free = k == 1 || cin < 256 || cout < 256;
        double best = -1.0;
        std::pair<int, int> pick(ks0, 0);
        for (int ks = 1; ks <= cap; ks++) {
            const long long chunk = ((M + ks - 1) / ks + 63) / 64 * 64;
            if ((long long)(ks - 1) * chunk >= M) continue;
            const double tw = (chunk / 64 + 8) * 2.3;
            const double tail = 3.0 + 2.4 * ks * ((double)cout * k * k * cin / (512.0 * 4608.0));
            const double t = makespan(nd, td, tiles * ks, tw) + tail;
            if (best < 0.0 || t < best) { best = t; pick = {ks, 0}; }
            if (order_free) {
                const double t2 = makespan(tiles * ks, tw, nd, td) + tail;
                if (t2 < best) { best = t2; pick = {ks, 1}; }
            }
        }
        return pick;
    });
}

struct DgradShape {
    int ngroups, B, H, W, kch, taps, tiles_m, tiles_n, xcd_mix, row_tiles, cls_tiles, skip_taps, grid, dil[4];
};
struct WgradShape {
    int ngroups, B, H, W, cin, cout, taps, tiles_n, tiles_c, ksplit, compact, xcd_mix, nent, grid, dil[4];
    const uint32_t *plan;
};

inline std::vector<int> tile_tap_list(int B, int H, int W, int d, int mode) {
    const long long M = (long long)B * H * W;
    std::vector<int> out;
    if (mode == 1) {
        const int r = kBM / W;
        for (int b = 0; b < B; b++)
            for (int y0 = 0; y0 < H; y0 += r) out.push_back(__builtin_popcount(tap_mask_rect(H, W, d, y0, std::min(H, y0 + r), 0, W)));
        return out;
    }
    HostClass c[kMaxClasses];
    const int n = mode == 2 ? build_classes(H, W, d, c) : 0;
    long long q0[kMaxClasses + 1] = {0};
    for (int k = 0; k < n; k++) q0[k + 1] = q0[k] + (long long)B * (c[k].y1 - c[k].y0) * (c[k].x1 - c[k].x0);
    for (long long t0 = 0; t0 < M; t0 += kBM) {
        const long long t1 = std::min(M, t0 + kBM);
        uint32_t m = 0;
        for (int k = 0; k < n; k++)
            if (q0[k] < t1 && q0[k + 1] > t0) m |= c[k].mask;
        for (long long p = t0; mode == 0 && p < t1;) {
            const int rem = (int)(p % ((long long)H * W)), y = rem / W, x = rem % W;
            const int x1 = (int)std::min<long long>(W, x + (t1 - p));
            m |= tap_mask_rect(H, W, d, y, y + 1, x, x1);
            p += x1 - x;
        }
        out.push_back(__builtin_popcount(m));
    }
    return out;
}

inline DgradShape dgrad_shape_for(int ngroups, int B, int H, int W, int cin, int cout, int k, const int *dil, const IgemmVariant &v) {
    DgradShape s{};
    const long long M = (long long)B * H * W;
    s.ngroups = ngroups; s.B = B; s.H = H; s.W = W; s.kch = cout / 64; s.taps = k * k;
    s.tiles_m = (int)((M + kBM - 1) / kBM);
    s.tiles_n = (cin + kBN - 1) / kBN;
    s.skip_taps = v.skip_dead_steps;
    for (int g = 0; g < ngroups; g++) {
        s.dil[g] = dil ? dil[g] : 1;
        if (s.skip_taps && k == 3 && s.dil[g] >= 3) s.xcd_mix = 1;
    }
    const bool rows_ok = s.xcd_mix && W <= kBM && conv_igemm_row_tiles(H, W);
    if (s.xcd_mix && v.class_tiles_allowed && H <= 255 && W <= 255 && (class_order_pays(B, H, W, s.dil, ngroups, rows_ok) || v.class_tiles_forced))
        s.cls_tiles = 1;
    if (!s.cls_tiles && rows_ok) {
        s.row_tiles = 1;
        s.tiles_m = B * ((H + kBM / W - 1) / (kBM / W));
    }
    s.grid = s.xcd_mix ? 8 * ngroups * ((s.tiles_m + 7) / 8) * s.tiles_n : s.tiles_m * s.tiles_n * ngroups;
    return s;
}
inline WgradShape wgrad_shape_for(int ngroups, int B, int H, int W, int cin, int cout, int k, const int *dil, const IgemmVariant &v,
                                  int forced_ksplit, int cus) {
    WgradShape s{};
    const long long M = (long long)B * H * W;
    s.ngroups = ngroups; s.B = B; s.H = H; s.W = W; s.cin = cin; s.cout = cout; s.taps = k * k;
    s.tiles_n = (cout + 255) / 256;
    s.tiles_c = wgrad_col_tiles(cin, k);
    for (int q = 0; q < ngroups; q++) s.dil[q] = dil ? dil[q] : 1;
    const WgradPlan *p = (forced_ksplit <= 0 && wgrad_wants_plan(v, dil, ngroups, cin, k)) ? &build_wgrad_plan(ngroups, B, H, W, cin, cout, dil, cus) : nullptr;
    s.ksplit = forced_ksplit > 0 ? forced_ksplit : wgrad_uniform_ksplit(ngroups, M, cin, cout, k, wgrad_wants_mix(dil, ngroups, k));
    for (int q = 0; q < ngroups; q++) {
        if (v.skip_dead_steps && k == 3 && s.dil[q] >= 3 &&
            (s.ksplit % 8 == 0 || (8 % s.ksplit == 0 && (s.tiles_n * s.tiles_c) % (8 / s.ksplit) == 0))) s.xcd_mix = 1;
        if (v.skip_dead_steps && v.wgrad_compact && k == 3 && cin != 128 && s.dil[q] >= 1) s.compact = 1;
    }
    s.grid = s.tiles_n * s.tiles_c * s.ksplit * ngroups;
    if (p) {
        s.plan = p->words.data();
        s.nent = p->nent;
        s.grid = (s.nent + 7) / 8 * 8 * (s.tiles_n * ((cin + 255) / 256));
    }
    return s;
}

inline bool dgrad_block_tile(const DgradShape &s, int id, int &grp, int &tm, int &tn) {
    const int xcd = id & 7, k = id >> 3;
    if (s.xcd_mix) {
        const int cm = (s.tiles_m - xcd + 7) >> 3, per_group = cm * s.tiles_n;
        if (cm <= 0 || k >= per_group * s.ngroups) return false;
        grp = k / per_group;
        const int r = k - grp * per_group, tml = r / s.tiles_n;
        tn = r - tml * s.tiles_n;
        tm = xcd + 8 * tml;
        return true;
    }
    const int q = s.grid >> 3, r = s.grid & 7, per_group = s.tiles_m * s.tiles_n;
    int t = (xcd < r ? xcd * (q + 1) : r * (q + 1) + (xcd - r) * q) + k;
    grp = t / per_group;
    t -= grp * per_group;
    tm = t / s.tiles_n;
    tn = t - tm * s.tiles_n;
    return true;
}
inline bool wgrad_block_unit(const WgradShape &s, int id, int &grp, int &split, int &ksp, int &t) {
    const int xcd = id & 7, k = id >> 3, tiles = s.tiles_n * s.tiles_c;
    ksp = s.ksplit;
    if (s.plan) {
        const int ncb = (s.cin + 255) >> 8, tpe = s.tiles_n * ncb, pos = k / tpe, te = k - pos * tpe, e = pos * 8 + xcd;
        if (e >= s.nent) return false;
        const uint32_t w = s.plan[kPlanHdr + e];
        grp = (int)(w & 3u);
        split = (int)((w >> 6) & 255u);
        ksp = (int)((w >> 14) & 255u);
        t = (te / ncb) * s.tiles_c + (int)((w >> 2) & 15u) * ncb + te % ncb;
    } else if (s.xcd_mix && s.ksplit >= 8) {
        const int per_group = (s.ksplit >> 3) * tiles;
        grp = k / per_group;
        const int r = k - grp * per_group;
        split = xcd + 8 * (r / tiles);
        t = r % tiles;
    } else if (s.xcd_mix) {
        const int xpc = 8 / s.ksplit, per_group = tiles / xpc;
        split = xcd / xpc;
        grp = k / per_group;
        t = xcd % xpc + xpc * (k - grp * per_group);
    } else {
        const int q = s.grid >> 3, r = s.grid & 7, tiles_per_group = tiles * s.ksplit;
        t = (xcd < r ? xcd * (q + 1) : r * (q + 1) + (xcd - r) * q) + k;
        grp = t / tiles_per_group;
        t -= grp * tiles_per_group;
        split = t / tiles;
        t -= split * tiles;
    }
    return true;
}

inline std::vector<double> dgrad_block_costs(const DgradShape &s) {
    std::vector<std::vector<int>> live(s.ngroups);
    for (int g = 0; g < s.ngroups; g++) {
        if (s.taps == 9 && s.skip_taps) live[g] = tile_tap_list(s.B, s.H, s.W, s.dil[g], s.cls_tiles ? 2 : s.row_tiles ? 1 : 0);
        else live[g].assign((size_t)s.tiles_m, s.taps);
    }
    std::vector<double> c((size_t)std::max(s.grid, 0), 0.0);
    for (int id = 0; id < s.grid; id++) {
        int grp, tm, tn;
        if (dgrad_block_tile(s, id, grp, tm, tn)) c[(size_t)id] = (s.kch * live[grp][(size_t)tm] + 6) * 1.85;
    }
    return c;
}
inline std::vector<double> wgrad_block_costs(const WgradShape &s) {
    std::vector<double> c((size_t)std::max(s.grid, 0), 0.0);
    const long long M = (long long)s.B * s.H * s.W;
    const bool two = s.cin == 128 && s.taps == 9;
    const int ncb = two ? 1 : (s.cin + 255) >> 8;
    for (int id = 0; id < s.grid; id++) {
        int grp, split, ksp, t;
        if (!wgrad_block_unit(s, id, grp, split, ksp, t)) continue;
        const int tc = t % s.tiles_c, tap = two ? 2 * tc : tc / ncb;
        long long Kc = M, chunk = ((M + s.ksplit - 1) / s.ksplit + 63) / 64 * 64;
        if (s.compact && !two && s.taps == 9) {
            const int rh = s.H - abs((tap / 3 - 1) * s.dil[grp]), rw = s.W - abs((tap % 3 - 1) * s.dil[grp]);
            Kc = (rh > 0 && rw > 0) ? (long long)s.B * rh * rw : 0;
            chunk = ((Kc + ksp - 1) / ksp + 63) / 64 * 64;
        }
        const long long beg = split * chunk, end = std::min(Kc, beg + chunk);
        c[(size_t)id] = ((end > beg ? (end - beg + 63) / 64 : 0) + 8) * 2.3;
    }
    return c;
}

inline int merged_second_half_start(int n_first) { return (n_first + 7) & ~7; }
inline double merged_grid_makespan(const std::vector<double> &first, const std::vector<double> &second, int cus) {
    const size_t n0 = first.size(), pad = (size_t)merged_second_half_start((int)n0);
    return dispatch_makespan(cus, [&](int x, int b) {
        const size_t id = (size_t)x + 8 * (size_t)b;
        if (id < n0) return first[id];
        if (id < pad) return 0.0;
        return id - pad < second.size() ? second[id - pad] : -1.0;
    });
}

struct MergedGroupsPlan {
    bool merge;
    int w_first;
    int ksplit;
    double merged_us, separate_us;
};
inline MergedGroupsPlan merged_groups_decide(const std::vector<double> &dcost, const std::vector<double> &wcost, int cus) {
    MergedGroupsPlan p{false, 0, 0, 0.0, 0.0};
    const std::vector<double> none;
    p.separate_us = merged_grid_makespan(dcost, none, cus) + merged_grid_makespan(wcost, none, cus);
    p.merged_us = p.separate_us;
    if (dcost.empty() || wcost.empty()) return p;
    const double d_first = merged_grid_makespan(dcost, wcost, cus), w_first = merged_grid_makespan(wcost, dcost, cus);
    p.w_first = w_first < d_first || (w_first == d_first && *std::max_element(wcost.begin(), wcost.end()) > *std::max_element(dcost.begin(), dcost.end()));
    p.merged_us = std::min(d_first, w_first);
    p.merge = p.merged_us <= p.separate_us;
    if (!p.merge) p.merged_us = p.separate_us;
    return p;
}
inline const MergedGroupsPlan &merged_groups_plan(const DgradShape &d, int cin, int cout, int k, const IgemmVariant &v, int forced_ksplit, int cus) {
    static PlanMemo<std::array<int, 20>, MergedGroupsPlan> memo;
    const int vbits = v.skip_dead_steps | v.class_tiles_allowed << 1 | v.class_tiles_forced << 2 | v.wgrad_work_list << 3 | v.wgrad_compact << 4;
    const std::array<int, 20> key = {d.ngroups, d.B, d.H, d.W, cin, cout, k, d.dil[0], d.dil[1], d.dil[2], d.dil[3], d.tiles_m, d.xcd_mix,
                                     d.row_tiles, d.cls_tiles, d.skip_taps, d.grid, vbits, forced_ksplit, cus};
    return memo.get(key, [&] {
        const long long M = (long long)d.B * d.H * d.W;
        const std::vector<double> dcost = dgrad_block_costs(d);
        const WgradShape w0 = wgrad_shape_for(d.ngroups, d.B, d.H, d.W, cin, cout, k, d.dil, v, 0, cus);
        auto priced = [&](const WgradShape &w) {
            double planes = (double)w.ksplit * w.taps * d.ngroups;
            if (w.plan) { planes = 0.0; for (int i = 0; i < d.ngroups * 9; i++) planes += (double)w.plan[2 * i]; }
            const double tail = 3.0 + 2.4 * planes * ((double)cout * cin / (512.0 * 4608.0));
            MergedGroupsPlan p = merged_groups_decide(dcost, wgrad_block_costs(w), cus);
            p.merged_us += tail;
            p.separate_us += tail;
            p.ksplit = w.plan ? 0 : w.ksplit;
            return p;
        };
        MergedGroupsPlan best = priced(w0);
        const double separate = best.separate_us;
        if (!w0.plan && (forced_ksplit > 0 || !wgrad_wants_mix(d.dil, d.ngroups, k))) {
            const int bound = wgrad_ksplit_bound(d.ngroups, d.B, d.H, d.W, cin, cout, k);
            for (int ks = 1; ks <= bound; ks++) {
                if ((long long)(ks - 1) * (((M + ks - 1) / ks + 63) / 64 * 64) >= M) continue;
                if (forced_ksplit > 0 ? ks != forced_ksplit : ks == w0.ksplit) continue;
                const MergedGroupsPlan p = priced(wgrad_shape_for(d.ngroups, d.B, d.H, d.W, cin, cout, k, d.dil, v, ks, cus));
                if (forced_ksplit > 0 || (p.merge && p.merged_us < best.merged_us)) best = p;
            }
        }
        if (forced_ksplit <= 0) {
            best.separate_us = separate;
            best.merge = best.merge && best.merged_us <= separate;
            if (!best.merge) { best.merged_us = separate; best.ksplit = w0.plan ? 0 : w0.ksplit; }
        }
        return best;
    });
}

}
```

dsrg_amd/ops.py:

```python
import contextlib
import ctypes
import os
import threading
import weakref as _weakref

import torch

from . import _lib
from ._lib import CrfParams, check
from .crf import select_arrays


def _stream():
    return ctypes.c_void_p(torch.cuda.current_stream().cuda_stream)


def _ptr(t):
    return ctypes.c_void_p(t.data_ptr()) if t is not None else None


def _f32c(t, name):
    if not (t.is_cuda and t.dtype == torch.float32 and t.is_contiguous()):
        raise ValueError("%s must be a contiguous float32 CUDA tensor" % name)
    return t
# ... 670 lines not shown
        check(_lib.lib().dsrg_bias_grad_bf16(_ptr(g), _ptr(gb), _ptr(part), _PARTIAL_BLOCKS, B * H * W, C, _stream()))
    return gb


def avgpool3x3_s1(x):
    B, C, H, W = x.shape
    x = x.contiguous(memory_format=torch.channels_last)
    out = torch.empty_like(x)
    check(_lib.lib().dsrg_avgpool3x3_s1_bf16(_ptr(x), _ptr(out), B, H, W, C, _stream()))
    return out


def add_relu(a, b):
    if not (a.is_cuda and a.dtype == torch.bfloat16 and b.dtype == torch.bfloat16 and a.shape == b.shape and a.numel() % 8 == 0):
        raise ValueError("add_relu needs two bf16 CUDA tensors of one shape, 8 | elements")
    if a.stride() != b.stride() or not (a.is_contiguous() or a.is_contiguous(memory_format=torch.channels_last)):
        a, b = a.contiguous(memory_format=torch.channels_last), b.contiguous(memory_format=torch.channels_last)
    y = torch.empty_like(a)
    check(_lib.lib().dsrg_add_relu_bf16(_ptr(a), _ptr(b), _ptr(y), a.numel(), _stream()))
    return y


def relu_mask(g, y, g2=None):
    if not (y.is_cuda and y.dtype == torch.bfloat16 and g.dtype == torch.bfloat16 and g.shape == y.shape and y.numel() % 8 == 0):
        raise ValueError("relu_mask needs bf16 CUDA tensors of one shape, 8 | elements")
    if not (y.is_contiguous() or y.is_contiguous(memory_format=torch.channels_last)):
        raise ValueError("relu_mask: y must be dense")
    mf = torch.contiguous_format if y.is_contiguous() else torch.channels_last

    def dense(t):
        return t if t.stride() == y.stride() else t.contiguous(memory_format=mf)
    g = dense(g)
    g2 = dense(g2) if g2 is not None else None
    gm = torch.empty_like(y)
    check(_lib.lib().dsrg_relu_mask_bf16(_ptr(g), _ptr(g2) if g2 is not None else None, _ptr(y), _ptr(gm), y.numel(), _stream()))
    return gm


DIRECT_CONV_CHANNELS = (64, 128)


def conv3x3_direct(x, weight, bias=None, relu=False):
    B, C, H, W = x.shape
    cl = torch.channels_last
    cout = weight.shape[0]
    if not (x.is_cuda and x.dtype == torch.bfloat16 and weight.dtype == torch.bfloat16 and tuple(weight.shape) == (cout, C, 3, 3)
            and ((C in DIRECT_CONV_CHANNELS and cout in DIRECT_CONV_CHANNELS) or (C, cout) == (3, 64))):
        raise ValueError("conv3x3_direct needs a bf16 CUDA input and a (cout,cin,3,3) bf16 kernel with cin, cout in (64, 128) or 3 -> 64")
    x = x.contiguous(memory_format=cl)
    w = weight.contiguous(memory_format=cl)
    if bias is not None:
        bias = bias.float().contiguous()
    y = torch.empty((B, cout, H, W), dtype=torch.bfloat16, device=x.device, memory_format=cl)
    check(_lib.lib().dsrg_conv3x3_direct_bf16(_ptr(x), _ptr(w), _ptr(bias), _ptr(y), B, H, W, C, cout, int(bool(relu)), _stream()))
    return y


def conv3x3_direct_dgrad(g, weight_t, mask):
    B, C, H, W = g.shape
    cl = torch.channels_last
    cout = weight_t.shape[0]
    if not (g.is_cuda and g.dtype == torch.bfloat16 and weight_t.dtype == torch.bfloat16 and tuple(weight_t.shape) == (cout, C, 3, 3)
            and C in DIRECT_CONV_CHANNELS and cout in DIRECT_CONV_CHANNELS and mask.dtype == torch.bfloat16
            and tuple(mask.shape) == (B, cout, H, W) and mask.is_contiguous(memory_format=cl)):
        raise ValueError("conv3x3_direct_dgrad needs bf16 CUDA tensors, 64 / 128 channels, a channels_last mask of the output's shape")
    g = g.contiguous(memory_format=cl)
    w = weight_t.contiguous(memory_format=cl)
    L = _lib.lib()
    gx = torch.empty((B, cout, H, W), dtype=torch.bfloat16, device=g.device, memory_format=cl)
    gb = _bias_grad_dest(None, (cout,), g.device)
    ws = _reduction_scratch(g.device, L.dsrg_conv3x3_direct_dgrad_workspace(cout))
    check(L.dsrg_conv3x3_direct_dgrad_bf16(_ptr(g), _ptr(w), _ptr(mask), _ptr(gx), _ptr(gb), _ptr(ws), ws.numel(), B, H, W, C, cout,
                                           _stream()))
    return gx, gb


WGRAD_CONV_SHAPES = ((3, 64), (64, 64), (64, 128), (128, 128))


class _KeptPacks(object):
    __slots__ = ("owner", "kind", "at", "version", "fwd", "dg")

    def __init__(self, owner):
        self.owner = _weakref.ref(owner)
        self.forget()

    def forget(self):
        self.kind = self.at = self.version = self.fwd = self.dg = None


def _lies(weight):
    return weight.data_ptr(), tuple(weight.shape), tuple(weight.stride())


def keep_weight_packs(params, owner):
    for p in params:
        p._dsrg_packs = _KeptPacks(owner) if owner is not None else None


def forget_weight_packs(params):
    for p in params:
        if getattr(p, "_dsrg_packs", None) is not None:
            p._dsrg_packs.forget()


def _packs_claimed(weight):
    r = getattr(weight, "_dsrg_packs", None)
    return r is not None and r.owner() is not None


def kept_packs(weight, kind=None):
    r = getattr(weight, "_dsrg_packs", None)
    if r is None or r.kind is None:
        return None
    if r.owner() is None or r.at != _lies(weight) or (kind is not None and r.kind != kind):
        r.forget()
        return None
    return r


def _packs_keep(weight, kind, fwd, dg):
    r = weight._dsrg_packs
    r.kind, r.at, r.version, r.fwd, r.dg = kind, _lies(weight), weight._version, fwd, dg


_CHECK_PACKS = int(os.environ.get("DSRG_CHECK_PACKS", "0") or 0)
_check_packs_calls = [0]


def _check_kept_packs(weight, fwd, dg, pack):
    if _CHECK_PACKS <= 0:
        return
    _check_packs_calls[0] += 1
    if _check_packs_calls[0] % _CHECK_PACKS:
        return
    f2 = torch.empty_like(fwd) if fwd is not None else None
    d2 = torch.empty_like(dg) if dg is not None else None
    pack(f2, d2)
    if (f2 is not None and not torch.equal(f2, fwd)) or (d2 is not None and not torch.equal(d2, dg)):
        raise RuntimeError("DSRG_CHECK_PACKS: the kept bf16 kernels of a %s parameter no longer match its float32 value — it was "
                           "written behind the version counter's back (param.data, a foreign kernel, torch._fused_sgd_); call "
                           "dsrg_amd.ops.forget_weight_packs([param]) after such a write" % (tuple(weight.shape),))


def _kept_or_packed(weight, kind, want_fwd, want_dgrad, fwd_shape, dg_shape, mf, pack):
    keep = _packs_claimed(weight) and weight.is_cuda and not torch.cuda.is_current_stream_capturing()
    r = kept_packs(weight, kind) if keep else None
    fwd, dg = (r.fwd, r.dg) if r is not None else (None, None)
    if r is not None and r.version == weight._version and (fwd is not None or not want_fwd) and (dg is not None or not want_dgrad):
        _check_kept_packs(weight, fwd if want_fwd else None, dg if want_dgrad else None, pack)
    else:
        if fwd is None and want_fwd:
            fwd = torch.empty(fwd_shape, dtype=torch.bfloat16, device=weight.device, memory_format=mf)
        if dg is None and want_dgrad:
            dg = torch.empty(dg_shape, dtype=torch.bfloat16, device=weight.device, memory_format=mf)
        pack(fwd, dg)
        if keep:
            _packs_keep(weight, kind, fwd, dg)
    return (fwd if want_fwd else None), (dg if want_dgrad else None)


def sgd_pack_step(params, grads, bufs, lrs, wds, momentum):
    import numpy as np
    n = len(params)
    if n == 0:
        return
    ptr = lambda ts: np.array([0 if t is None else t.data_ptr() for t in ts], dtype=np.uint64)
    fwd, dg, cast, shape, entries = [None] * n, [None] * n, [None] * n, np.zeros((n, 4), dtype=np.int32), []
    for i, p in enumerate(params):
        e = kept_packs(p)
        if e is None:
            continue
        if e.kind == "cast":
            cast[i] = e.fwd
        else:
            fwd[i], dg[i] = e.fwd, e.dg
            shape[i] = (p.shape[0], p.shape[1], p.shape[2] * p.shape[3], int(e.kind == "direct"))
        entries.append((e, p))
    pp, gp, bp, fp, dp, cp = ptr(params), ptr(grads), ptr(bufs), ptr(fwd), ptr(dg), ptr(cast)
    numel = np.array([p.numel() for p in params], dtype=np.int64)
    lr, wd = np.asarray(lrs, dtype=np.float32), np.asarray(wds, dtype=np.float32)
    a = lambda x: x.ctypes.data
    check(_lib.lib().dsrg_sgd_pack_cast_f32(n, a(pp), a(gp), a(bp), a(fp), a(dp), a(cp), a(shape), a(numel), a(lr), a(wd),
                                            float(momentum), _stream()))
    torch.autograd.graph.increment_version(list(params))
    for e, p in entries:
        e.version = p._version


def sgd_pack_eligible(p, g, b):
    return p.is_cuda and p.dtype == torch.float32 and g.dtype == torch.float32 and b.dtype == torch.float32 and g.is_cuda and \
        g.shape == p.shape and all(n == 1 or (sg == sp and sb == sp) for n, sp, sg, sb in zip(p.shape, p.stride(), g.stride(), b.stride())) and \
        (p.is_contiguous() or (p.dim() == 4 and p.is_contiguous(memory_format=torch.channels_last))) and \
        ((p.data_ptr() | b.data_ptr()) % 16 == 0 or kept_packs(p) is None)


def cast_weight_kept(weight):
    w = weight.detach()
    dense = w.is_contiguous() or (w.dim() == 4 and w.is_contiguous(memory_format=torch.channels_last))
    if not (w.dtype == torch.float32 and dense):
        return w.to(torch.bfloat16)
    mf = torch.contiguous_format if w.is_contiguous() else torch.channels_last
    return _kept_or_packed(weight, "cast", True, False, w.shape, None, mf, lambda f, d: f.copy_(w))[0]


def pack_direct_weight_pair(weight, want_dgrad=True):
    cout, cin = weight.shape[0], weight.shape[1]
    cl = torch.channels_last
    if not (weight.is_cuda and weight.dtype == torch.float32 and weight.is_contiguous(memory_format=cl) and tuple(weight.shape[2:]) == (3, 3)
            and cin in DIRECT_CONV_CHANNELS and cout in DIRECT_CONV_CHANNELS):
        raise ValueError("pack_direct_weight_pair needs a float32 channels_last (cout,cin,3,3) CUDA parameter with 64 / 128 channels")
    pack = lambda f, d: check(_lib.lib().dsrg_pack_conv_weight_direct_f32(_ptr(weight.detach()), _ptr(f), _ptr(d), cout, cin, _stream()))
    return _kept_or_packed(weight, "direct", True, want_dgrad, (cout, cin, 3, 3), (cin, cout, 3, 3), cl, pack)


def conv3x3_wgrad(x, g, out_dtype=torch.bfloat16, out=None):
    B, cin, H, W = x.shape
    cout = g.shape[1]
    cl = torch.channels_last
    if not (x.is_cuda and x.dtype == torch.bfloat16 and g.dtype == torch.bfloat16 and tuple(g.shape) == (B, cout, H, W)
            and (cin, cout) in WGRAD_CONV_SHAPES):
        raise ValueError("conv3x3_wgrad needs bf16 CUDA tensors with (cin, cout) in %s" % (WGRAD_CONV_SHAPES,))
    x = x.contiguous(memory_format=cl)
    g = g.contiguous(memory_format=cl)
    ws = _stream_scratch("wgrad3x3", x.device, _lib.lib().dsrg_conv3x3_wgrad_workspace(B, H, W, cin, cout))
    if out_dtype not in (torch.bfloat16, torch.float32):
        raise ValueError("conv3x3_wgrad: bf16 or float32 output")
    gw = _dest(out, (cout, cin, 3, 3), out_dtype, x.device, True)
    fn = _lib.lib().dsrg_conv3x3_wgrad_f32 if out_dtype == torch.float32 else _lib.lib().dsrg_conv3x3_wgrad_bf16
    check(fn(_ptr(x), _ptr(g), _ptr(gw), _ptr(ws), ws.numel(), B, H, W, cin, cout, _stream()))
    return gw


def conv_igemm_supported(cin, cout, k):
    return bool(_lib.lib().dsrg_conv_igemm_supported(int(cin), int(cout), int(k)))


def set_igemm_variant(v):
    _lib.lib().dsrg_debug_set_igemm_variant(int(v))


def pack_conv_weight(weight, for_dgrad=False, dtype=torch.bfloat16):
    k = weight.shape[2]
    if for_dgrad:
        weight = weight.flip(2, 3).transpose(0, 1) if k > 1 else weight.transpose(0, 1)
    o, c = weight.shape[0], weight.shape[1]
    out = torch.empty((o, c // 64, k * k, 64), dtype=dtype, device=weight.device)
    if weight.is_contiguous(memory_format=torch.channels_last) and not weight.is_contiguous():
        out.copy_(weight.permute(0, 2, 3, 1).reshape(o, k * k, c // 64, 64).permute(0, 2, 1, 3))
    else:
        out.copy_(weight.reshape(o, c // 64, 64, k * k).permute(0, 1, 3, 2))
    return out


def pack_conv_weight_pair(weight, want_fwd=True, want_dgrad=True, scale=None):
    cout, cin, k, _ = weight.shape
    if scale is not None:
        if not (weight.is_cuda and weight.dtype == torch.float32 and weight.is_contiguous(memory_format=torch.channels_last)
                and cout % 64 == 0 and cin % 64 == 0 and k in (1, 3)):
            return pack_conv_weight_pair((weight.detach() * scale.view(-1, 1, 1, 1)).contiguous(memory_format=torch.channels_last), want_fwd, want_dgrad)
        fwd = torch.empty((cout, cin // 64, k * k, 64), dtype=torch.bfloat16, device=weight.device) if want_fwd else None
        dg = torch.empty((cin, cout // 64, k * k, 64), dtype=torch.bfloat16, device=weight.device) if want_dgrad else None
        check(_lib.lib().dsrg_pack_conv_weight_scaled_f32(_ptr(weight.detach()), _ptr(_f32c(scale, "scale")), _ptr(fwd), _ptr(dg), cout, cin, k,
                                                          _stream()))
        return fwd, dg
    if not (weight.is_cuda and weight.dtype == torch.float32 and weight.is_contiguous(memory_format=torch.channels_last)
            and cout % 64 == 0 and cin % 64 == 0 and k in (1, 3)):
        return (pack_conv_weight(weight) if want_fwd else None, pack_conv_weight(weight, for_dgrad=True) if want_dgrad else None)
    pack = lambda f, d: check(_lib.lib().dsrg_pack_conv_weight_f32(_ptr(weight.detach()), _ptr(f), _ptr(d), cout, cin, k, _stream()))
    return _kept_or_packed(weight, "igemm", want_fwd, want_dgrad, (cout, cin // 64, k * k, 64), (cin, cout // 64, k * k, 64),
                           torch.contiguous_format, pack)


def split3_bf16(t, dim):
    p0 = t.to(torch.bfloat16)
    r1 = t - p0.float()
    p1 = r1.to(torch.bfloat16)
    p2 = (r1 - p1.float()).to(torch.bfloat16)
    return torch.cat([p0, p1, p2], dim=dim)


def conv_igemm_split(x, weight, bias, dilation, relu):
    B, cin, H, W = x.shape
    cout, k = weight.shape[0], weight.shape[2]
    x3 = split3_bf16(x.permute(0, 2, 3, 1).contiguous().float(), 3)
    w0, w1, w2 = [pack_conv_weight(p) for p in split3_bf16(weight.float(), 0).split(cout, 0)]
    wv = torch.cat([w0, w1, w0, w2, w0, w1], dim=1).contiguous()
    y = torch.empty((B, cout, H, W), dtype=torch.float32, device=x.device, memory_format=torch.channels_last)
    b = bias.float().contiguous() if bias is not None else None
    check(_lib.lib().dsrg_conv_igemm_split_f32(_ptr(x3), _ptr(wv), _ptr(b), _ptr(y), int(dilation), B, H, W, cin, cout, k, int(bool(relu)),
                                               _stream()))
    return y


def _is_bf16(t, shape, channels_last=False):
    return (t.is_cuda and t.dtype == torch.bfloat16 and tuple(t.shape) == tuple(shape)
            and (not channels_last or t.is_contiguous(memory_format=torch.channels_last)))


def _is_packed(p, rows, chunk_channels, ksize):
    return p.dtype == torch.bfloat16 and tuple(p.shape) == (rows, chunk_channels // 64, ksize * ksize, 64) and p.is_contiguous()


def conv_igemm(xs, packed, biases, dilations, ksize, relu, dropout_p=0.0, seed=0, stream_k=True):
    n = len(xs)
    B, cin, H, W = xs[0].shape
    cout = packed[0].shape[0]
    cl = torch.channels_last
    if not (1 <= n <= 4 and len(packed) == n and len(dilations) == n):
        raise ValueError("conv_igemm: 1..4 groups")
    if not all(_is_bf16(x, (B, cin, H, W)) and _is_packed(p, cout, cin, ksize) for x, p in zip(xs, packed)):
        raise ValueError("conv_igemm needs bf16 CUDA inputs of one shape and kernels packed by pack_conv_weight")
    xs = [x.contiguous(memory_format=cl) for x in xs]
    bs = [None if b is None else _f32c(b, "bias") for b in (biases or [None] * n)]
    ys = [torch.empty((B, cout, H, W), dtype=torch.bfloat16, device=xs[0].device, memory_format=cl) for _ in range(n)]
    ws = _igemm_sk_workspace(xs[0].device) if stream_k else None
    check(_lib.lib().dsrg_conv_igemm_bf16(_ptrs(xs), _ptrs(packed), _ptrs(bs), _ptrs(ys), _i32s(dilations), n, B, H, W, cin, cout, ksize,
                                          int(bool(relu)), float(dropout_p), int(seed) & 0xFFFFFFFFFFFFFFFF, _ptr(ws),
                                          ws.numel() if ws is not None else 0, _stream()))
    return ys


def conv_igemm_residual(x, packed, bias, res, mask, dilation, ksize, relu):
    B, cin, H, W = x.shape
    cout = packed.shape[0]
    cl = torch.channels_last
    if not (_is_bf16(x, x.shape) and _is_packed(packed, cout, cin, ksize) and _is_bf16(res, (B, cout, H, W), True)
            and (mask is None or _is_bf16(mask, (B, cout, H, W), True))):
        raise ValueError("conv_igemm_residual needs bf16 channels_last tensors of matching shapes and a kernel packed by pack_conv_weight")
    x = x.contiguous(memory_format=cl)
    b = None if bias is None else _f32c(bias, "bias")
    y = torch.empty((B, cout, H, W), dtype=torch.bfloat16, device=x.device, memory_format=cl)
    check(_lib.lib().dsrg_conv_igemm_residual_bf16(_ptr(x), _ptr(packed), _ptr(b), _ptr(res), _ptr(mask), _ptr(y), int(dilation), B, H, W,
                                                   cin, cout, ksize, int(bool(relu)), _stream()))
    return y


def aspp_shift_sum(y, offsets, outputs, bias=None):
    B, CT, H, W = y.shape
    J = len(offsets)
    if not (y.is_cuda and y.dtype == torch.bfloat16 and y.is_contiguous(memory_format=torch.channels_last) and 1 <= J <= 36 and J * outputs <= CT):
        raise ValueError("aspp_shift_sum needs a bf16 channels_last (B,CT,H,W) tensor with CT >= pairs * outputs, at most 36 pairs")
    out = torch.empty((B, H, W, outputs), dtype=torch.float32, device=y.device)
    off = (ctypes.c_int * (2 * J))(*[int(v) for pair in offsets for v in pair])
    b = None if bias is None else _f32c(bias, "bias")
    check(_lib.lib().dsrg_aspp_shift_sum_f32(_ptr(y), _ptr(b), _ptr(out), off, J, int(outputs), CT, B, H, W, _stream()))
    return out.permute(0, 3, 1, 2)


def aspp_shift_gather(g, offsets, channels):
    B, O, H, W = g.shape
    J = len(offsets)
    if not (g.is_cuda and 1 <= J <= 36 and J * O <= channels):
        raise ValueError("aspp_shift_gather: at most 36 pairs, channels >= pairs * outputs")
    gn = g.float().permute(0, 2, 3, 1).contiguous()
    gp = torch.empty((B, channels, H, W), dtype=torch.bfloat16, device=g.device, memory_format=torch.channels_last)
    off = (ctypes.c_int * (2 * J))(*[int(v) for pair in offsets for v in pair])
    check(_lib.lib().dsrg_aspp_shift_gather_bf16(_ptr(gn), _ptr(gp), off, J, O, int(channels), B, H, W, _stream()))
    return gp


def conv_igemm_dgrad(gs, packed_t, masks, dilations, ksize, mask_scale=1.0, bias_grad=True, gb_outs=None):
    n = len(gs)
    B, cin, H, W = gs[0].shape
    cout = packed_t[0].shape[0]
    cl = torch.channels_last
    if not (1 <= n <= 4 and len(packed_t) == n and len(dilations) == n and len(masks) == n):
        raise ValueError("conv_igemm_dgrad: 1..4 groups")
    if not all(_is_bf16(g, (B, cin, H, W)) and _is_packed(p, cout, cin, ksize) and _is_bf16(m, (B, cout, H, W), True)
               for g, p, m in zip(gs, packed_t, masks)):
        raise ValueError("conv_igemm_dgrad needs bf16 channels_last gradients / masks of one shape and packed kernels")
    gs = [g.contiguous(memory_format=cl) for g in gs]
    outs = [torch.empty((B, cout, H, W), dtype=torch.bfloat16, device=gs[0].device, memory_format=cl) for _ in range(n)]
    L = _lib.lib()
    gb = ws = None
    if bias_grad:
        gb = [_bias_grad_dest(gb_outs[i] if gb_outs is not None else None, (cout,), gs[0].device) for i in range(n)]
        ws = _reduction_scratch(gs[0].device, L.dsrg_conv_igemm_dgrad_workspace(n, B, H, W, cout))
    check(L.dsrg_conv_igemm_dgrad_bf16(_ptrs(gs), _ptrs(packed_t), _ptrs(masks), _ptrs(outs), _ptrs(gb), _i32s(dilations), n, B, H, W, cin,
                                       cout, ksize, float(mask_scale), _ptr(ws), ws.numel() if ws is not None else 0, _stream()))
    return outs, gb


def _conv_igemm_backward_args(name, g, packed_d, x, ksize, gw_out, **like_x):
    B, cout, H, W = g.shape
    cin = x.shape[1]
    cl = torch.channels_last
    if not (_is_bf16(g, g.shape) and _is_bf16(x, (B, cin, H, W), True) and _is_packed(packed_d, cin, cout, ksize)
            and all(t is None or _is_bf16(t, (B, cin, H, W), True) for t in like_x.values())):
        raise ValueError("%s needs bf16 channels_last g / x (/ %s) of one geometry and the data-gradient packing" % (name, " / ".join(like_x)))
    g = g.contiguous(memory_format=cl)
    L = _lib.lib()
    need = L.dsrg_conv_igemm_wgrad_workspace(1, B, H, W, cin, cout, ksize)
    if need == 0:
        raise ValueError("%s: 256 | cin (or cin = 128 with a 3x3 kernel), 256 | cout required (got %d, %d)" % (name, cin, cout))
    ws = _stream_scratch("igemm_wgrad", g.device, need)
    gx = torch.empty((B, cin, H, W), dtype=torch.bfloat16, device=g.device, memory_format=cl)
    gw = _dest(gw_out, (cout, cin, ksize, ksize), torch.float32, g.device, True)
    return L, g, ws, gx, gw, (B, H, W, cin, cout, ksize)


def conv_igemm_backward(g, packed_d, x, dilation, mask=None, mask_scale=1.0, ksize=3, gw_out=None, gb_out=None):
    L, g, ws, gx, gw, geom = _conv_igemm_backward_args("conv_igemm_backward", g, packed_d, x, ksize, gw_out, mask=mask)
    B, H, W, cin = geom[:4]
    gb = cws = None
    if mask is not None:
        gb = _bias_grad_dest(gb_out, (cin,), g.device)
        cws = _reduction_scratch(g.device, L.dsrg_conv_igemm_dgrad_workspace(1, B, H, W, cin))
    check(L.dsrg_conv_igemm_backward_bf16(_ptr(g), _ptr(packed_d), _ptr(x), _ptr(mask), _ptr(gx), _ptr(gw), int(dilation), _ptr(gb),
                                          float(mask_scale), _ptr(cws), cws.numel() if cws is not None else 0, _ptr(ws), ws.numel(),
                                          *geom, _stream()))
    return gx, gw, gb


def conv_igemm_backward_residual(g, packed_d, x, dilation, ksize, mask=None, res=None, gw_scale=None, gw_out=None):
    L, g, ws, gx, gw, geom = _conv_igemm_backward_args("conv_igemm_backward_residual", g, packed_d, x, ksize, gw_out, mask=mask, res=res)
    sc = None if gw_scale is None else _f32c(gw_scale, "gw_scale")
    check(L.dsrg_conv_igemm_backward_residual_bf16(_ptr(g), _ptr(packed_d), _ptr(x), _ptr(mask), _ptr(res), _ptr(gx), _ptr(gw), _ptr(sc),
                                                   int(dilation), _ptr(ws), ws.numel(), *geom, _stream()))
    return gx, gw


def conv_igemm_backward_groups(gs, packed_d, xs, dilations, ksize, masks=None, mask_scale=1.0, gw_outs=None, gb_outs=None, gx_outs=None,
                               force_ksplit=0, force_order=0):
    n = len(gs)
    B, cout, H, W = gs[0].shape
    cin = xs[0].shape[1]
    cl = torch.channels_last
    if not (1 <= n <= 4 and len(packed_d) == n and len(xs) == n and len(dilations) == n and (masks is None or len(masks) == n)):
        raise ValueError("conv_igemm_backward_groups: 1..4 groups")
    if not all(_is_bf16(gs[i], (B, cout, H, W)) and _is_bf16(xs[i], (B, cin, H, W), True) and _is_packed(packed_d[i], cin, cout, ksize)
               and (masks is None or _is_bf16(masks[i], (B, cin, H, W), True)) for i in range(n)):
        raise ValueError("conv_igemm_backward_groups needs bf16 channels_last g / x (/ mask) of one geometry and the data-gradient packing")
    gs = [g.contiguous(memory_format=cl) for g in gs]
    dev = gs[0].device
    L = _lib.lib()
    need = L.dsrg_conv_igemm_wgrad_workspace(n, B, H, W, cin, cout, ksize)
    if need == 0 or not conv_igemm_supported(cout, cin, ksize):
        raise ValueError("conv_igemm_backward_groups: 64 | cout, 128 | cin, k in (1, 3) required (got %d, %d, %d)" % (cout, cin, ksize))
    ws = _stream_scratch("igemm_wgrad", dev, need)
    gxs = [_dest(gx_outs[i] if gx_outs is not None else None, (B, cin, H, W), torch.bfloat16, dev, True) for i in range(n)]
    gws = [_dest(gw_outs[i] if gw_outs is not None else None, (cout, cin, ksize, ksize), torch.float32, dev, True) for i in range(n)]
    gbs = cws = None
    if masks is not None:
        gbs = [_bias_grad_dest(gb_outs[i] if gb_outs is not None else None, (cin,), dev) for i in range(n)]
        cws = _reduction_scratch(dev, L.dsrg_conv_igemm_dgrad_workspace(n, B, H, W, cin))
    check(L.dsrg_conv_igemm_backward_groups_bf16(_ptrs(gs), _ptrs(packed_d), _ptrs(xs), _ptrs(masks), _ptrs(gxs), _ptrs(gws), _i32s(dilations), n,
                                                 _ptrs(gbs), float(mask_scale), _ptr(cws), cws.numel() if cws is not None else 0, _ptr(ws),
                                                 ws.numel(), B, H, W, cin, cout, ksize, int(force_ksplit), int(force_order), _stream()))
    return gxs, gws, gbs


def conv_igemm_backward_groups_plan(n, B, H, W, cin, cout, ksize, dilations, with_mask=False, force_ksplit=0, force_order=0):
    out = (ctypes.c_int * 5)()
    us = (ctypes.c_double * 2)()
    check(_lib.lib().dsrg_conv_igemm_backward_groups_plan(int(n), int(B), int(H), int(W), int(cin), int(cout), int(ksize),
                                                           (ctypes.c_int * n)(*[int(d) for d in dilations]), int(bool(with_mask)),
                                                           int(force_ksplit), int(force_order), out, us))
    return {"merged": bool(out[0]), "w_first": bool(out[1]), "ksplit": out[2], "nd": out[3], "nw": out[4],
            "merged_us": us[0], "separate_us": us[1]}


def _igemm_sk_workspace(device):
    return _stream_scratch("igemm_stream_k", device, _lib.lib().dsrg_conv_igemm_workspace())


def conv_igemm_stream_k_status(device=None):
    device = device or torch.device("cuda", torch.cuda.current_device())
    ws = _igemm_sk_workspace(device)
    st = ctypes.c_int(0)
    check(_lib.lib().dsrg_conv_igemm_workspace_status(_ptr(ws), _stream(), ctypes.byref(st)))
    return st.value


def dropout_seed():
    return int(torch.randint(0, 2 ** 62, (1,), dtype=torch.int64).item())


def conv_igemm_wgrad_supported(cin, cout, k):
    cin, cout, k = int(cin), int(cout), int(k)
    return k in (1, 3) and ((cin >= 256 and cin % 256 == 0) or (cin == 128 and k == 3)) and cout >= 256 and cout % 256 == 0


def conv_igemm_wgrad_launchable(cin, cout, k):
    return _lib.lib().dsrg_conv_igemm_wgrad_workspace(1, 1, 8, 8, int(cin), int(cout), int(k)) > 0


def conv_igemm_wgrad(xs, gs, dilations, ksize, out_dtype=torch.float32, outs=None):
    n = len(xs)
    B, cin, H, W = xs[0].shape
    cout = gs[0].shape[1]
    cl = torch.channels_last
    if not (1 <= n <= 4 and len(gs) == n and len(dilations) == n) or out_dtype not in (torch.float32, torch.bfloat16):
        raise ValueError("conv_igemm_wgrad: 1..4 groups, float32 or bfloat16 result")
    if not all(_is_bf16(x, (B, cin, H, W)) and _is_bf16(g, (B, cout, H, W)) for x, g in zip(xs, gs)):
        raise ValueError("conv_igemm_wgrad needs bf16 CUDA tensors of one geometry")
    xs = [x.contiguous(memory_format=cl) for x in xs]
    gs = [g.contiguous(memory_format=cl) for g in gs]
    L = _lib.lib()
    need = L.dsrg_conv_igemm_wgrad_workspace(n, B, H, W, cin, cout, ksize)
    if need == 0:
        raise ValueError("conv_igemm_wgrad: 64 | cin, 64 | cout, k in (1, 3) required (got %d, %d, %d)" % (cin, cout, ksize))
    ws = _stream_scratch("igemm_wgrad", xs[0].device, need)
    gws = [_dest(outs[i] if outs is not None else None, (cout, cin, ksize, ksize), out_dtype, xs[0].device, True) for i in range(n)]
    check(L.dsrg_conv_igemm_wgrad_bf16(_ptrs(xs), _ptrs(gs), _ptrs(gws), _i32s(dilations), n, _ptr(ws), ws.numel(), B, H, W, cin, cout, ksize,
                                       int(out_dtype == torch.bfloat16), _stream()))
    return gws


def conv_igemm_wgrad_splits(n, B, H, W, cin, cout, ksize, dilations):
    taps = int(ksize) * int(ksize)
    out = (ctypes.c_int * (n * taps))()
    check(_lib.lib().dsrg_conv_igemm_wgrad_splits(int(n), int(B), int(H), int(W), int(cin), int(cout), int(ksize),
                                                   (ctypes.c_int * n)(*[int(d) for d in dilations]), out))
    return [list(out[g * taps:(g + 1) * taps]) for g in range(n)]


def heads_forward(xs, weight, bias):
    B, K, H, W = xs[0].shape
    n, O = weight.shape[0], weight.shape[1]
    cl = torch.channels_last
    xs = [x.contiguous(memory_format=cl) for x in xs]
    if not all(x.is_cuda and x.dtype == torch.bfloat16 and x.shape == xs[0].shape for x in xs) or len(xs) != n:
        raise ValueError("heads_forward needs n bf16 CUDA activations of one shape")
    _f32c(weight, "weight")
    if bias is not None:
        _f32c(bias, "bias")
    out = torch.empty((B, O, H, W), dtype=torch.float32, device=xs[0].device)
    ptrs = (ctypes.c_void_p * 4)(*([x.data_ptr() for x in xs] + [None] * (4 - n)))
    check(_lib.lib().dsrg_heads_forward_bf16(ptrs, n, _ptr(weight), _ptr(bias), _ptr(out), B, H * W, K, O, _stream()))
    return out


def heads_backward(xs, weight, g, need_gx=True, relu_scale=0.0):
    B, K, H, W = xs[0].shape
    n, O = weight.shape[0], weight.shape[1]
    cl = torch.channels_last
    xs = [x.contiguous(memory_format=cl) for x in xs]
    _f32c(weight, "weight")
    g = g.contiguous()
    _f32c(g, "g")
    L = _lib.lib()
    M = B * H * W
    gx = torch.empty((n, B, H, W, K), dtype=torch.bfloat16, device=g.device) if need_gx else None
    gw = torch.empty((n, O, K), dtype=torch.float32, device=g.device)
    part = torch.empty(L.dsrg_heads_backward_chunks(M) * n * O * K, dtype=torch.float32, device=g.device)
    ptrs = (ctypes.c_void_p * 4)(*([x.data_ptr() for x in xs] + [None] * (4 - n)))
    if relu_scale > 0.0 and need_gx:
        gb = _bias_grad_dest(None, (n, K), g.device)
        ws = _reduction_scratch(g.device, L.dsrg_heads_backward_relu_workspace(n, M, K))
        check(L.dsrg_heads_backward_relu_bf16(ptrs, n, _ptr(weight), _ptr(g), _ptr(gx), M * K * 2, _ptr(gw), _ptr(part),
                                              float(relu_scale), _ptr(gb), _ptr(ws), ws.numel(), B, H * W, K, O, _stream()))
        return [gx[k].permute(0, 3, 1, 2) for k in range(n)], gw, gb
    check(L.dsrg_heads_backward_bf16(ptrs, n, _ptr(weight), _ptr(g), _ptr(gx), M * K * 2, _ptr(gw), _ptr(part), B, H * W, K, O,
                                     _stream()))
    return ([gx[k].permute(0, 3, 1, 2) for k in range(n)] if need_gx else None), gw


def _vp4(ts):
    return (ctypes.c_void_p * 4)(*([t.data_ptr() for t in ts] + [None] * (4 - len(ts))))


def heads_kernels_in_place(weights, biases=None):
    if not 1 <= len(weights) <= 4 or weights[0].dim() < 2:
        return False
    O, K = weights[0].shape[0], weights[0].shape[1]
    if not all(w.is_cuda and w.dtype == torch.float32 and w.shape == weights[0].shape and w.numel() == O * K and w.is_contiguous()
               for w in weights):
        return False
    return biases is None or (len(biases) == len(weights) and all(
        b.is_cuda and b.dtype == torch.float32 and tuple(b.shape) == (O,) and b.is_contiguous() for b in biases))


def heads_forward_ptrs(xs, weights, biases):
    B, K, H, W = xs[0].shape
    n, O = len(weights), weights[0].shape[0]
    cl = torch.channels_last
    xs = [x.contiguous(memory_format=cl) for x in xs]
    if not all(x.is_cuda and x.dtype == torch.bfloat16 and x.shape == xs[0].shape for x in xs) or len(xs) != n:
        raise ValueError("heads_forward_ptrs needs n bf16 CUDA activations of one shape")
    if not heads_kernels_in_place(weights, biases) or weights[0].shape[1] != K:
        raise ValueError("heads_forward_ptrs needs n float32 CUDA kernels whose memory is (O,K) row-major, and (O) biases")
    out = torch.empty((B, O, H, W), dtype=torch.float32, device=xs[0].device)
    check(_lib.lib().dsrg_heads_forward_ptrs_bf16(_vp4(xs), n, _vp4(weights), _vp4(biases) if biases is not None else None, _ptr(out),
                                                  B, H * W, K, O, _stream()))
    return out


def heads_backward_ptrs(xs, weights, g, need_gx=True, relu_scale=0.0, gw_outs=None):
    B, K, H, W = xs[0].shape
    n, O = len(weights), weights[0].shape[0]
    cl = torch.channels_last
    xs = [x.contiguous(memory_format=cl) for x in xs]
    if not heads_kernels_in_place(weights) or weights[0].shape[1] != K:
        raise ValueError("heads_backward_ptrs needs n float32 CUDA kernels whose memory is (O,K) row-major")
    g = g.contiguous()
    _f32c(g, "g")
    L = _lib.lib()
    M = B * H * W
    gx = torch.empty((n, B, H, W, K), dtype=torch.bfloat16, device=g.device) if need_gx else None
    gws = []
    for k, w in enumerate(weights):
        out = gw_outs[k] if gw_outs is not None else None
        if out is not None and out.dtype == torch.float32 and out.shape == w.shape and out.device == w.device and out.is_contiguous():
            gws.append(out)
        else:
            gws.append(torch.empty_strided(tuple(w.shape), tuple(w.stride()), dtype=torch.float32, device=g.device))
    part = torch.empty(L.dsrg_heads_backward_chunks(M) * n * O * K, dtype=torch.float32, device=g.device)
    masked = relu_scale > 0.0 and need_gx
    gb = _bias_grad_dest(None, (n, K), g.device) if masked else None
    ws = _reduction_scratch(g.device, L.dsrg_heads_backward_relu_workspace(n, M, K)) if masked else None
    check(L.dsrg_heads_backward_ptrs_bf16(_vp4(xs), n, _vp4(weights), _ptr(g), _ptr(gx), M * K * 2, _vp4(gws), _ptr(part),
                                          float(relu_scale) if masked else 0.0, _ptr(gb), _ptr(ws), ws.numel() if masked else 0,
                                          B, H * W, K, O, _stream()))
    gxs = [gx[k].permute(0, 3, 1, 2) for k in range(n)] if need_gx else None
    return (gxs, gws, gb) if masked else (gxs, gws)


def image_to_bf16_nhwc(x):
    if not (x.dim() == 4 and x.shape[1] == 3):
        raise ValueError("image_to_bf16_nhwc needs a (B,3,H,W) image")
    _f32c(x, "x")
    B, _, H, W = x.shape
    y = torch.empty((B, 3, H, W), dtype=torch.bfloat16, device=x.device, memory_format=torch.channels_last)
    check(_lib.lib().dsrg_image_nchw_to_nhwc_bf16(_ptr(x), _ptr(y), B, H, W, _stream()))
    return y


def image_takes_fused_cast(x):
    return x.is_cuda and x.dtype == torch.float32 and x.dim() == 4 and x.shape[1] == 3 and x.is_contiguous() and x.numel() > 0


def sum_bf16(ts):
    t0 = ts[0]
    if not (2 <= len(ts) <= 4 and all(t.is_cuda and t.dtype == torch.bfloat16 and t.shape == t0.shape and t.stride() == t0.stride()
                                      for t in ts) and t0.numel() % 8 == 0 and t0.numel() > 0 and
            (t0.is_contiguous() or (t0.dim() == 4 and t0.is_contiguous(memory_format=torch.channels_last)))):
        raise ValueError("sum_bf16 needs 2..4 dense bf16 CUDA tensors of one shape and layout, 8 | elements")
    out = torch.empty_like(t0)
    check(_lib.lib().dsrg_sum_bf16(_vp4(ts), len(ts), _ptr(out), t0.numel(), _stream()))
    return out


def maxpool3x3_out_size(n, stride, ceil_mode):
    num = n + 2 - 3
    o = (-(-num // stride) if ceil_mode else num // stride) + 1
    if (o - 1) * stride >= n + 1:
        o -= 1
    return o


def resnet_stem_pack(weight, scale):
    if not (weight.is_cuda and weight.dtype == torch.float32 and tuple(weight.shape) == (64, 3, 7, 7)):
        raise ValueError("resnet_stem_pack needs a (64,3,7,7) float32 CUDA kernel")
    if tuple(scale.shape) != (64,):
        raise ValueError("resnet_stem_pack needs 64 scales")
    w = weight.detach().contiguous()
    nbytes = _lib.lib().dsrg_resnet_stem_packed_bytes()
    packed = torch.empty((64, nbytes // 128), dtype=torch.bfloat16, device=weight.device)
    check(_lib.lib().dsrg_pack_resnet_stem_f32(_ptr(w), _ptr(_f32c(scale.detach(), "scale")), _ptr(packed), _stream()))
    return packed


def resnet_stem(x, packed, shift):
    if not (x.dim() == 4 and x.shape[1] == 3):
        raise ValueError("resnet_stem needs a (B,3,H,W) input")
    x = _f32c(x, "x")
    B, _, H, W = x.shape
    if not (packed.is_cuda and packed.dtype == torch.bfloat16 and packed.is_contiguous()
            and packed.numel() * 2 == _lib.lib().dsrg_resnet_stem_packed_bytes()):
        raise ValueError("resnet_stem needs a kernel packed by resnet_stem_pack")
    if tuple(shift.shape) != (64,):
        raise ValueError("resnet_stem needs 64 shifts")
    OHc, OWc = (H - 1) // 2 + 1, (W - 1) // 2 + 1
    PH, PW = maxpool3x3_out_size(OHc, 2, True), maxpool3x3_out_size(OWc, 2, True)
    y = torch.empty((B, 64, PH, PW), dtype=torch.bfloat16, device=x.device, memory_format=torch.channels_last)
# ... 61 lines not shown
```

Baseline: 2102.

## Balance igemm tile work across XCDs with planner-built greedy assignment tables

Adds a host-side greedy longest-processing-time assignment that maps tiles (dgrad) and plan entries (wgrad) to the 8 XCDs by estimated cost. The tables are passed as kernel arguments to new template variants that look up each block's tile, and are used in both the forward igemm and the merged backward kernel. In the merged backward case the table also accounts for load already placed by the other half. This targets uneven per-XCD work from skipped taps and compact wgrad, at the cost of larger kernel arguments, extra kernel variants and reliance on a cost model. It also adds optional preallocated output arguments in the Python ops.

New measurement: 2116 (median of 6 runs). No clear change (+0.7%).

```diff
diff --git a/dsrg_amd/csrc/conv_igemm.hip b/dsrg_amd/csrc/conv_igemm.hip
--- a/dsrg_amd/csrc/conv_igemm.hip
+++ b/dsrg_amd/csrc/conv_igemm.hip
@@ -64,6 +64,15 @@
     int out_f32;
     int cls_tiles;
 };
+struct XcdTiles {
+    int xrows;
+    uint32_t xtab[kXcdTileSlots / 2];
+};
+struct XcdEntries {
+    int xrows;
+    uint32_t xtab[kXcdEntrySlots / 2];
+};
+__device__ __forceinline__ uint32_t xcd_slot(const uint32_t *tab, int s) { return (tab[s >> 1] >> ((s & 1) << 4)) & 0xffffu; }
 
 __device__ __forceinline__ uint32_t fmix32(uint32_t h) {
     h ^= h >> 16; h *= 0x85EBCA6Bu; h ^= h >> 13; h *= 0xC2B2AE35u; h ^= h >> 16;
@@ -117,7 +126,8 @@
     }
 }
 
-__device__ __forceinline__ void conv_igemm_body(const IgemmArgs &a, const int bid, const int nblk) {
+template <bool XTAB>
+__device__ __forceinline__ void conv_igemm_body(const IgemmArgs &a, const XcdTiles *xt, const int bid, const int nblk) {
     using C = ICfg<64, 2>;
     extern __shared__ __attribute__((aligned(16))) unsigned char ig_lds[];
     const int tid = threadIdx.x, lane = tid & 63;
@@ -126,7 +136,15 @@
     const int wn = wv >> 2, wm = wv & 3;
 
     int grp, tm, tn;
-    if (a.xcd_mix) {
+    if (XTAB && a.xcd_mix && xt->xrows > 0) {
+        const int xcd = bid & 7, k = bid >> 3, pos = k / a.tiles_n;
+        if (pos >= xt->xrows) return;
+        const int u = (int)xcd_slot(xt->xtab, pos * 8 + xcd);
+        if (u == (int)kXcdHole) return;
+        grp = u / a.tiles_m;
+        tm = u - grp * a.tiles_m;
+        tn = k - pos * a.tiles_n;
+    } else if (a.xcd_mix) {
         const int id = bid, xcd = id & 7, k = id >> 3;
         const int cm = (a.tiles_m - xcd + 7) >> 3, per_group = cm * a.tiles_n;
         if (cm <= 0 || k >= per_group * a.ngroups) return;
@@ -430,7 +448,9 @@
 }
 
 
-__global__ __launch_bounds__(512, 2) void conv_igemm_kernel_64x2(IgemmArgs a) { conv_igemm_body(a, (int)blockIdx.x, (int)gridDim.x); }
+__global__ __launch_bounds__(512, 2) void conv_igemm_kernel_64x2(IgemmArgs a) { conv_igemm_body<false>(a, nullptr, (int)blockIdx.x, (int)gridDim.x); }
+struct IgemmXcdArgs { IgemmArgs a; XcdTiles x; };
+__global__ __launch_bounds__(512, 2) void conv_igemm_xcd_kernel(IgemmXcdArgs k) { conv_igemm_body<true>(k.a, &k.x, (int)blockIdx.x, (int)gridDim.x); }
 
 struct IgemmSkArgs {
     IgemmArgs base;
@@ -673,7 +693,8 @@
     return __builtin_shufflevector(lo, hi, 0, 1, 2, 3, 4, 5, 6, 7);
 }
 
-__device__ __forceinline__ void conv_igemm_wgrad_body(const IgemmWgradArgs &a, const int bid, const int nblk) {
+template <bool XTAB>
+__device__ __forceinline__ void conv_igemm_wgrad_body(const IgemmWgradArgs &a, const XcdEntries *xe, const int bid, const int nblk) {
     extern __shared__ __attribute__((aligned(16))) unsigned char ig_lds[];
     const int tid = threadIdx.x, lane = tid & 63;
     const int wv = __builtin_amdgcn_readfirstlane(tid >> 6);
@@ -685,7 +706,9 @@
     size_t plane = 0;
     if (a.plan) {
         const int ncb_ = (a.Cin + 255) >> 8, tpe = a.tiles_n * ncb_;
-        const int xcd = bid & 7, k = bid >> 3, pos = k / tpe, te = k - pos * tpe, e = pos * 8 + xcd;
+        const int xcd = bid & 7, k = bid >> 3, pos = k / tpe, te = k - pos * tpe;
+        int e = pos * 8 + xcd;
+        if (XTAB && xe->xrows > 0) e = pos < xe->xrows ? (int)xcd_slot(xe->xtab, e) : (int)kXcdHole;
         if (e >= a.nent) return;
         const uint32_t w = a.plan[kPlanHdr + e];
         grp = (int)(w & 3u);
@@ -877,7 +900,7 @@
         }
 }
 
-__global__ __launch_bounds__(512, 2) void conv_igemm_wgrad_kernel(IgemmWgradArgs a) { conv_igemm_wgrad_body(a, (int)blockIdx.x, (int)gridDim.x); }
+__global__ __launch_bounds__(512, 2) void conv_igemm_wgrad_kernel(IgemmWgradArgs a) { conv_igemm_wgrad_body<false>(a, nullptr, (int)blockIdx.x, (int)gridDim.x); }
 
 struct IgemmBwdArgs {
     IgemmArgs d;
@@ -889,16 +912,35 @@
     const int id = (int)blockIdx.x;
     if (a.w_first) {
         if (id < a.nw_pad) {
-            if (id < a.nw) conv_igemm_wgrad_body(a.w, id, a.nw);
+            if (id < a.nw) conv_igemm_wgrad_body<false>(a.w, nullptr, id, a.nw);
         } else if (id - a.nw_pad < a.nd) {
-            conv_igemm_body(a.d, id - a.nw_pad, a.nd);
+            conv_igemm_body<false>(a.d, nullptr, id - a.nw_pad, a.nd);
         }
         return;
     }
     if (id < a.nd_pad) {
-        if (id < a.nd) conv_igemm_body(a.d, id, a.nd);
+        if (id < a.nd) conv_igemm_body<false>(a.d, nullptr, id, a.nd);
     } else {
-        conv_igemm_wgrad_body(a.w, id - a.nd_pad, a.nw);
+        conv_igemm_wgrad_body<false>(a.w, nullptr, id - a.nd_pad, a.nw);
+    }
+}
+struct IgemmBwdXcdArgs { IgemmBwdArgs b; XcdTiles xd; XcdEntries xw; };
+static_assert(sizeof(IgemmBwdXcdArgs) <= 4096, "a kernel's arguments hold 4 KB: both halves with their XCD tables");
+__global__ __launch_bounds__(512, 2) void conv_igemm_bwd_xcd_kernel(IgemmBwdXcdArgs k) {
+    const IgemmBwdArgs &a = k.b;
+    const int id = (int)blockIdx.x;
+    if (a.w_first) {
+        if (id < a.nw_pad) {
+            if (id < a.nw) conv_igemm_wgrad_body<true>(a.w, &k.xw, id, a.nw);
+        } else if (id - a.nw_pad < a.nd) {
+            conv_igemm_body<true>(a.d, &k.xd, id - a.nw_pad, a.nd);
+        }
+        return;
+    }
+    if (id < a.nd_pad) {
+        if (id < a.nd) conv_igemm_body<true>(a.d, &k.xd, id, a.nd);
+    } else {
+        conv_igemm_wgrad_body<true>(a.w, &k.xw, id - a.nd_pad, a.nw);
     }
 }
 
@@ -1028,8 +1070,19 @@
 }
 
 namespace {
+int put_xcd_table(XcdTiles &x, const DgradShape &s) {
+    x.xrows = s.xrows;
+    if (s.xrows > 0) memcpy(x.xtab, s.xtab, (size_t)s.xrows * 8 * sizeof(uint16_t));
+    return s.grid;
+}
+int put_xcd_table(XcdEntries &x, const WgradShape &s) {
+    x.xrows = s.xrows;
+    if (s.xrows > 0) memcpy(x.xtab, s.xtab, (size_t)s.xrows * 8 * sizeof(uint16_t));
+    return s.grid;
+}
 struct IgemmLaunch {
     IgemmSkArgs sk;
+    XcdTiles x;
     int grid;
     bool stream_k;
 };
@@ -1121,6 +1174,12 @@
         a.tiles_per_group = a.tiles_m * a.tiles_n;
     }
     L.grid = a.xcd_mix ? 8 * ngroups * ((a.tiles_m + 7) / 8) * a.tiles_n : a.tiles_per_group * ngroups;
+    if (a.xcd_mix && v.xcd_balance) {
+        const DgradShape s = dgrad_shape_for(ngroups, B, H, W, cout, cin, k, dils, v);
+        if (s.tiles_m != a.tiles_m || s.tiles_n != a.tiles_n || s.xcd_mix != a.xcd_mix || s.row_tiles != a.row_tiles || s.cls_tiles != a.cls_tiles)
+            return set_error(DSRG_ERR_INVALID, "conv_igemm: the planner and the launcher disagree on the tiles");
+        L.grid = put_xcd_table(L.x, s);
+    }
     return DSRG_OK;
 }
 
@@ -1132,7 +1191,7 @@
 }
 
 int run_igemm(const IgemmLaunch &L, float *const *colsum, hipStream_t stream) {
-    static LdsGrant grant[2];
+    static LdsGrant grant[3];
     constexpr size_t lds = ICfg<64, 2>::LDS;
     const IgemmArgs &a = L.sk.base;
     if (L.stream_k) {
@@ -1142,8 +1201,16 @@
         DSRG_LAUNCH_CHECK();
         return DSRG_OK;
     }
-    if (int rc = ensure_dynamic_lds(reinterpret_cast<const void *>(&conv_igemm_kernel_64x2), lds, grant[0])) return rc;
-    hipLaunchKernelGGL(conv_igemm_kernel_64x2, dim3(L.grid), dim3(512), lds, stream, a);
+    if (L.x.xrows > 0) {
+        if (int rc = ensure_dynamic_lds(reinterpret_cast<const void *>(&conv_igemm_xcd_kernel), lds, grant[2])) return rc;
+        IgemmXcdArgs k;
+        k.a = a;
+        k.x = L.x;
+        hipLaunchKernelGGL(conv_igemm_xcd_kernel, dim3(L.grid), dim3(512), lds, stream, k);
+    } else {
+        if (int rc = ensure_dynamic_lds(reinterpret_cast<const void *>(&conv_igemm_kernel_64x2), lds, grant[0])) return rc;
+        hipLaunchKernelGGL(conv_igemm_kernel_64x2, dim3(L.grid), dim3(512), lds, stream, a);
+    }
     DSRG_LAUNCH_CHECK();
     return run_colsum(a, colsum, stream);
 }
@@ -1197,6 +1264,7 @@
 struct WgradLaunch {
     IgemmWgradArgs a;
     const WgradPlan *plan;
+    XcdEntries x;
     int grid;
 };
 
@@ -1302,11 +1370,21 @@
     return run_wgrad(L, r.gw, nullptr, out_bf16, stream);
 }
 
-static int launch_bwd_grid(const IgemmBwdArgs &a, hipStream_t stream) {
-    static LdsGrant grant;
+static int launch_bwd_grid(const IgemmBwdArgs &a, const XcdTiles &xd, const XcdEntries &xw, hipStream_t stream) {
+    static LdsGrant grant[2];
     constexpr size_t lds = ICfg<64, 2>::LDS > (size_t)(2 * kWStage) ? ICfg<64, 2>::LDS : (size_t)(2 * kWStage);
-    if (int rc = ensure_dynamic_lds(reinterpret_cast<const void *>(&conv_igemm_bwd_kernel), lds, grant)) return rc;
-    hipLaunchKernelGGL(conv_igemm_bwd_kernel, dim3(a.w_first ? a.nw_pad + a.nd : a.nd_pad + a.nw), dim3(512), lds, stream, a);
+    const dim3 grid(a.w_first ? a.nw_pad + a.nd : a.nd_pad + a.nw);
+    if (xd.xrows > 0 || xw.xrows > 0) {
+        if (int rc = ensure_dynamic_lds(reinterpret_cast<const void *>(&conv_igemm_bwd_xcd_kernel), lds, grant[1])) return rc;
+        IgemmBwdXcdArgs k;
+        k.b = a;
+        k.xd = xd;
+        k.xw = xw;
+        hipLaunchKernelGGL(conv_igemm_bwd_xcd_kernel, grid, dim3(512), lds, stream, k);
+    } else {
+        if (int rc = ensure_dynamic_lds(reinterpret_cast<const void *>(&conv_igemm_bwd_kernel), lds, grant[0])) return rc;
+        hipLaunchKernelGGL(conv_igemm_bwd_kernel, grid, dim3(512), lds, stream, a);
+    }
     DSRG_LAUNCH_CHECK();
     return DSRG_OK;
 }
@@ -1372,6 +1450,13 @@
     }
     P.merge = plan.merge;
     P.w_first = plan.w_first;
+    if (P.merge && v.xcd_balance) {
+        const MergedHalves &h = merged_groups_halves(ds, cin, cout, k, v, plan.ksplit, plan.w_first, igemm_cus());
+        if (h.w.ksplit != P.w.a.ksplit || h.w.nent != P.w.a.nent || (h.w.plan != nullptr) != (P.w.plan != nullptr))
+            return set_error(DSRG_ERR_INVALID, "conv_igemm_backward_groups: the planner and the launcher disagree on the merged halves");
+        P.d.grid = put_xcd_table(P.d.x, h.d);
+        P.w.grid = put_xcd_table(P.w.x, h.w);
+    }
     return DSRG_OK;
 }
 
@@ -1387,7 +1472,7 @@
     a.w = P.w.a;
     a.nd = P.d.grid; a.nd_pad = merged_second_half_start(a.nd); a.nw = P.w.grid; a.nw_pad = merged_second_half_start(a.nw);
     a.w_first = P.w_first;
-    if (int rc = launch_bwd_grid(a, stream)) return rc;
+    if (int rc = launch_bwd_grid(a, P.d.x, P.w.x, stream)) return rc;
     if (int rc = run_colsum(a.d, bias_grad, stream)) return rc;
     return reduce_wgrad(a.w, gw, gw_scale, 0, stream);
 }
diff --git a/dsrg_amd/csrc/igemm_plan.h b/dsrg_amd/csrc/igemm_plan.h
--- a/dsrg_amd/csrc/igemm_plan.h
+++ b/dsrg_amd/csrc/igemm_plan.h
@@ -25,10 +25,12 @@
     bool wgrad_work_list;
     bool wgrad_compact;
     bool merged_backward;
+    bool xcd_balance;
 };
 inline IgemmVariant decode_igemm_variant(int v) {
-    const int e = (v < 0 || v == 2 || v == 5) ? 3 : v;
-    return IgemmVariant{e >= 3, e != 6, e == 3 || e == 8 || e == 9, e == 4, e != 8, e == 9, e != 6 && e != 7, e != 7, e == 3 || e == 1 || e == 8 || e == 9};
+    const int e = (v < 0 || v == 2 || v == 5 || v == 13) ? 3 : v;
+    return IgemmVariant{e >= 3, e != 6, e == 3 || e == 8 || e == 9, e == 4, e != 8, e == 9, e != 6 && e != 7, e != 7, e == 3 || e == 1 || e == 8 || e == 9,
+                        v != 13};
 }
 
 template <class Key, class Value> struct PlanMemo {
@@ -57,6 +59,41 @@
         }
     }
     return worst;
+}
+
+constexpr int kXcdTileSlots = 1024;
+constexpr int kXcdEntrySlots = 256;
+constexpr uint16_t kXcdHole = 0xffff;
+using XcdLoads = std::array<double, 8>;
+struct XcdTable {
+    std::vector<uint16_t> slot;
+    int rows = 0;
+    XcdLoads load{};
+};
+inline XcdTable xcd_balance(const std::vector<double> &unit_cost, const XcdLoads &base) {
+    std::vector<int> order(unit_cost.size());
+    for (size_t u = 0; u < order.size(); u++) order[u] = (int)u;
+    std::stable_sort(order.begin(), order.end(), [&](int x, int y) { return unit_cost[(size_t)x] > unit_cost[(size_t)y]; });
+    XcdTable t;
+    t.load = base;
+    std::array<std::vector<uint16_t>, 8> list;
+    for (int u : order) {
+        int x = 0;
+        for (int c = 1; c < 8; c++)
+            if (t.load[c] < t.load[x]) x = c;
+        list[x].push_back((uint16_t)u);
+        t.load[x] += unit_cost[(size_t)u];
+    }
+    for (int x = 0; x < 8; x++) t.rows = std::max(t.rows, (int)list[x].size());
+    t.slot.assign((size_t)t.rows * 8, kXcdHole);
+    for (int x = 0; x < 8; x++)
+        for (size_t pos = 0; pos < list[x].size(); pos++) t.slot[pos * 8 + x] = list[x][pos];
+    return t;
+}
+inline XcdLoads xcd_loads(const std::vector<double> &block_cost) {
+    XcdLoads l{};
+    for (size_t id = 0; id < block_cost.size(); id++) l[id & 7] += block_cost[id];
+    return l;
 }
 
 inline bool conv_igemm_launchable(int cin, int cout, int k) {
@@ -307,10 +344,14 @@
 
 struct DgradShape {
     int ngroups, B, H, W, kch, taps, tiles_m, tiles_n, xcd_mix, row_tiles, cls_tiles, skip_taps, grid, dil[4];
+    int balance, xrows;
+    const uint16_t *xtab;
 };
 struct WgradShape {
     int ngroups, B, H, W, cin, cout, taps, tiles_n, tiles_c, ksplit, compact, xcd_mix, nent, grid, dil[4];
     const uint32_t *plan;
+    int balance, xrows;
+    const uint16_t *xtab;
 };
 
 inline std::vector<int> tile_tap_list(int B, int H, int W, int d, int mode) {
@@ -342,6 +383,39 @@
     return out;
 }
 
+inline std::vector<double> dgrad_tile_costs(const DgradShape &s) {
+    std::vector<double> c((size_t)s.ngroups * (size_t)s.tiles_m);
+    for (int g = 0; g < s.ngroups; g++) {
+        std::vector<int> live;
+        if (s.taps == 9 && s.skip_taps) live = tile_tap_list(s.B, s.H, s.W, s.dil[g], s.cls_tiles ? 2 : s.row_tiles ? 1 : 0);
+        else live.assign((size_t)s.tiles_m, s.taps);
+        for (int tm = 0; tm < s.tiles_m; tm++) c[(size_t)g * s.tiles_m + tm] = (s.kch * live[(size_t)tm] + 6) * 1.85;
+    }
+    return c;
+}
+inline int dgrad_closed_grid(const DgradShape &s) {
+    return s.xcd_mix ? 8 * s.ngroups * ((s.tiles_m + 7) / 8) * s.tiles_n : s.tiles_m * s.tiles_n * s.ngroups;
+}
+inline DgradShape dgrad_shape_on(DgradShape s, const XcdLoads &base) {
+    s.xrows = 0;
+    s.xtab = nullptr;
+    s.grid = dgrad_closed_grid(s);
+    if (!s.balance || !s.xcd_mix || (long long)s.ngroups * s.tiles_m >= kXcdHole) return s;
+    static PlanMemo<std::pair<std::array<int, 15>, XcdLoads>, XcdTable> memo;
+    const std::array<int, 15> key = {s.ngroups, s.B, s.H, s.W, s.kch, s.taps, s.tiles_m, s.tiles_n, s.row_tiles, s.cls_tiles, s.skip_taps,
+                                     s.dil[0], s.dil[1], s.dil[2], s.dil[3]};
+    const XcdTable &t = memo.get(std::make_pair(key, base), [&] {
+        std::vector<double> unit = dgrad_tile_costs(s);
+        for (double &u : unit) u *= s.tiles_n;
+        return xcd_balance(unit, base);
+    });
+    if (t.rows < 1 || t.rows * 8 > kXcdTileSlots) return s;
+    s.xrows = t.rows;
+    s.xtab = t.slot.data();
+    s.grid = 8 * t.rows * s.tiles_n;
+    return s;
+}
+
 inline DgradShape dgrad_shape_for(int ngroups, int B, int H, int W, int cin, int cout, int k, const int *dil, const IgemmVariant &v) {
     DgradShape s{};
     const long long M = (long long)B * H * W;
@@ -360,9 +434,49 @@
         s.row_tiles = 1;
         s.tiles_m = B * ((H + kBM / W - 1) / (kBM / W));
     }
-    s.grid = s.xcd_mix ? 8 * ngroups * ((s.tiles_m + 7) / 8) * s.tiles_n : s.tiles_m * s.tiles_n * ngroups;
+    s.balance = v.xcd_balance && s.xcd_mix;
+    return dgrad_shape_on(s, XcdLoads{});
+}
+inline double wgrad_unit_us(const WgradShape &s, int grp, int split, int ksp, int t) {
+    const long long M = (long long)s.B * s.H * s.W;
+    const bool two = s.cin == 128 && s.taps == 9;
+    const int ncb = two ? 1 : (s.cin + 255) >> 8;
+    const int tc = t % s.tiles_c, tap = two ? 2 * tc : tc / ncb;
+    long long Kc = M, chunk = ((M + s.ksplit - 1) / s.ksplit + 63) / 64 * 64;
+    if (s.compact && !two && s.taps == 9) {
+        const int rh = s.H - abs((tap / 3 - 1) * s.dil[grp]), rw = s.W - abs((tap % 3 - 1) * s.dil[grp]);
+        Kc = (rh > 0 && rw > 0) ? (long long)s.B * rh * rw : 0;
+        chunk = ((Kc + ksp - 1) / ksp + 63) / 64 * 64;
+    }
+    const long long beg = split * chunk, end = std::min(Kc, beg + chunk);
+    return ((end > beg ? (end - beg + 63) / 64 : 0) + 8) * 2.3;
+}
+inline int wgrad_closed_grid(const WgradShape &s) {
+    return s.plan ? (s.nent + 7) / 8 * 8 * (s.tiles_n * ((s.cin + 255) / 256)) : s.tiles_n * s.tiles_c * s.ksplit * s.ngroups;
+}
+inline WgradShape wgrad_shape_on(WgradShape s, const XcdLoads &base, int cus) {
+    s.xrows = 0;
+    s.xtab = nullptr;
+    s.grid = wgrad_closed_grid(s);
+    if (!s.balance || !s.plan || s.nent < 1 || s.nent >= kXcdHole) return s;
+    static PlanMemo<std::pair<std::array<int, 12>, XcdLoads>, XcdTable> memo;
+    const std::array<int, 12> key = {s.ngroups, s.B, s.H, s.W, s.cin, s.cout, s.compact, s.dil[0], s.dil[1], s.dil[2], s.dil[3], cus};
+    const XcdTable &t = memo.get(std::make_pair(key, base), [&] {
+        const int ncb = (s.cin + 255) >> 8, tpe = s.tiles_n * ncb;
+        std::vector<double> unit((size_t)s.nent);
+        for (int e = 0; e < s.nent; e++) {
+            const uint32_t w = s.plan[kPlanHdr + e];
+            unit[(size_t)e] = tpe * wgrad_unit_us(s, (int)(w & 3u), (int)((w >> 6) & 255u), (int)((w >> 14) & 255u), (int)((w >> 2) & 15u) * ncb);
+        }
+        return xcd_balance(unit, base);
+    });
+    if (t.rows < 1 || t.rows * 8 > kXcdEntrySlots) return s;
+    s.xrows = t.rows;
+    s.xtab = t.slot.data();
+    s.grid = 8 * t.rows * (s.tiles_n * ((s.cin + 255) >> 8));
     return s;
 }
+
 inline WgradShape wgrad_shape_for(int ngroups, int B, int H, int W, int cin, int cout, int k, const int *dil, const IgemmVariant &v,
                                   int forced_ksplit, int cus) {
     WgradShape s{};
@@ -378,17 +492,26 @@
             (s.ksplit % 8 == 0 || (8 % s.ksplit == 0 && (s.tiles_n * s.tiles_c) % (8 / s.ksplit) == 0))) s.xcd_mix = 1;
         if (v.skip_dead_steps && v.wgrad_compact && k == 3 && cin != 128 && s.dil[q] >= 1) s.compact = 1;
     }
-    s.grid = s.tiles_n * s.tiles_c * s.ksplit * ngroups;
     if (p) {
         s.plan = p->words.data();
         s.nent = p->nent;
-        s.grid = (s.nent + 7) / 8 * 8 * (s.tiles_n * ((cin + 255) / 256));
-    }
+    }
+    s.balance = v.xcd_balance && p != nullptr;
+    s.grid = wgrad_closed_grid(s);
     return s;
 }
 
 inline bool dgrad_block_tile(const DgradShape &s, int id, int &grp, int &tm, int &tn) {
     const int xcd = id & 7, k = id >> 3;
+    if (s.xcd_mix && s.xrows > 0) {
+        const int pos = k / s.tiles_n;
+        if (pos >= s.xrows || s.xtab[pos * 8 + xcd] == kXcdHole) return false;
+        const int u = s.xtab[pos * 8 + xcd];
+        grp = u / s.tiles_m;
+        tm = u - grp * s.tiles_m;
+        tn = k - pos * s.tiles_n;
+        return true;
+    }
     if (s.xcd_mix) {
         const int cm = (s.tiles_m - xcd + 7) >> 3, per_group = cm * s.tiles_n;
         if (cm <= 0 || k >= per_group * s.ngroups) return false;
@@ -410,7 +533,9 @@
     const int xcd = id & 7, k = id >> 3, tiles = s.tiles_n * s.tiles_c;
     ksp = s.ksplit;
     if (s.plan) {
-        const int ncb = (s.cin + 255) >> 8, tpe = s.tiles_n * ncb, pos = k / tpe, te = k - pos * tpe, e = pos * 8 + xcd;
+        const int ncb = (s.cin + 255) >> 8, tpe = s.tiles_n * ncb, pos = k / tpe, te = k - pos * tpe;
+        int e = pos * 8 + xcd;
+        if (s.xrows > 0) e = pos < s.xrows && s.xtab[e] != kXcdHole ? (int)s.xtab[e] : s.nent;
         if (e >= s.nent) return false;
         const uint32_t w = s.plan[kPlanHdr + e];
         grp = (int)(w & 3u);
@@ -440,35 +565,19 @@
 }
 
 inline std::vector<double> dgrad_block_costs(const DgradShape &s) {
-    std::vector<std::vector<int>> live(s.ngroups);
-    for (int g = 0; g < s.ngroups; g++) {
-        if (s.taps == 9 && s.skip_taps) live[g] = tile_tap_list(s.B, s.H, s.W, s.dil[g], s.cls_tiles ? 2 : s.row_tiles ? 1 : 0);
-        else live[g].assign((size_t)s.tiles_m, s.taps);
-    }
+    const std::vector<double> tile = dgrad_tile_costs(s);
     std::vector<double> c((size_t)std::max(s.grid, 0), 0.0);
     for (int id = 0; id < s.grid; id++) {
         int grp, tm, tn;
-        if (dgrad_block_tile(s, id, grp, tm, tn)) c[(size_t)id] = (s.kch * live[grp][(size_t)tm] + 6) * 1.85;
+        if (dgrad_block_tile(s, id, grp, tm, tn)) c[(size_t)id] = tile[(size_t)grp * s.tiles_m + tm];
     }
     return c;
 }
 inline std::vector<double> wgrad_block_costs(const WgradShape &s) {
     std::vector<double> c((size_t)std::max(s.grid, 0), 0.0);
-    const long long M = (long long)s.B * s.H * s.W;
-    const bool two = s.cin == 128 && s.taps == 9;
-    const int ncb = two ? 1 : (s.cin + 255) >> 8;
     for (int id = 0; id < s.grid; id++) {
         int grp, split, ksp, t;
-        if (!wgrad_block_unit(s, id, grp, split, ksp, t)) continue;
-        const int tc = t % s.tiles_c, tap = two ? 2 * tc : tc / ncb;
-        long long Kc = M, chunk = ((M + s.ksplit - 1) / s.ksplit + 63) / 64 * 64;
-        if (s.compact && !two && s.taps == 9) {
-            const int rh = s.H - abs((tap / 3 - 1) * s.dil[grp]), rw = s.W - abs((tap % 3 - 1) * s.dil[grp]);
-            Kc = (rh > 0 && rw > 0) ? (long long)s.B * rh * rw : 0;
-            chunk = ((Kc + ksp - 1) / ksp + 63) / 64 * 64;
-        }
-        const long long beg = split * chunk, end = std::min(Kc, beg + chunk);
-        c[(size_t)id] = ((end > beg ? (end - beg + 63) / 64 : 0) + 8) * 2.3;
+        if (wgrad_block_unit(s, id, grp, split, ksp, t)) c[(size_t)id] = wgrad_unit_us(s, grp, split, ksp, t);
     }
     return c;
 }
@@ -490,24 +599,29 @@
     int ksplit;
     double merged_us, separate_us;
 };
-inline MergedGroupsPlan merged_groups_decide(const std::vector<double> &dcost, const std::vector<double> &wcost, int cus) {
+inline MergedGroupsPlan merged_groups_decide_orders(const std::vector<double> &d_alone, const std::vector<double> &w_behind,
+                                                    const std::vector<double> &w_alone, const std::vector<double> &d_behind, int cus) {
     MergedGroupsPlan p{false, 0, 0, 0.0, 0.0};
     const std::vector<double> none;
-    p.separate_us = merged_grid_makespan(dcost, none, cus) + merged_grid_makespan(wcost, none, cus);
+    p.separate_us = merged_grid_makespan(d_alone, none, cus) + merged_grid_makespan(w_alone, none, cus);
     p.merged_us = p.separate_us;
-    if (dcost.empty() || wcost.empty()) return p;
-    const double d_first = merged_grid_makespan(dcost, wcost, cus), w_first = merged_grid_makespan(wcost, dcost, cus);
-    p.w_first = w_first < d_first || (w_first == d_first && *std::max_element(wcost.begin(), wcost.end()) > *std::max_element(dcost.begin(), dcost.end()));
+    if (d_alone.empty() || w_alone.empty()) return p;
+    const double d_first = merged_grid_makespan(d_alone, w_behind, cus), w_first = merged_grid_makespan(w_alone, d_behind, cus);
+    p.w_first = w_first < d_first || (w_first == d_first && *std::max_element(w_alone.begin(), w_alone.end()) > *std::max_element(d_alone.begin(), d_alone.end()));
     p.merged_us = std::min(d_first, w_first);
     p.merge = p.merged_us <= p.separate_us;
     if (!p.merge) p.merged_us = p.separate_us;
     return p;
 }
+inline MergedGroupsPlan merged_groups_decide(const std::vector<double> &dcost, const std::vector<double> &wcost, int cus) {
+    return merged_groups_decide_orders(dcost, wcost, wcost, dcost, cus);
+}
 inline const MergedGroupsPlan &merged_groups_plan(const DgradShape &d, int cin, int cout, int k, const IgemmVariant &v, int forced_ksplit, int cus) {
-    static PlanMemo<std::array<int, 20>, MergedGroupsPlan> memo;
-    const int vbits = v.skip_dead_steps | v.class_tiles_allowed << 1 | v.class_tiles_forced << 2 | v.wgrad_work_list << 3 | v.wgrad_compact << 4;
-    const std::array<int, 20> key = {d.ngroups, d.B, d.H, d.W, cin, cout, k, d.dil[0], d.dil[1], d.dil[2], d.dil[3], d.tiles_m, d.xcd_mix,
-                                     d.row_tiles, d.cls_tiles, d.skip_taps, d.grid, vbits, forced_ksplit, cus};
+    static PlanMemo<std::array<int, 22>, MergedGroupsPlan> memo;
+    const int vbits = v.skip_dead_steps | v.class_tiles_allowed << 1 | v.class_tiles_forced << 2 | v.wgrad_work_list << 3 | v.wgrad_compact << 4 |
+                      v.xcd_balance << 5;
+    const std::array<int, 22> key = {d.ngroups, d.B, d.H, d.W, cin, cout, k, d.dil[0], d.dil[1], d.dil[2], d.dil[3], d.tiles_m, d.xcd_mix,
+                                     d.row_tiles, d.cls_tiles, d.skip_taps, d.grid, vbits, forced_ksplit, cus, d.balance, d.xrows};
     return memo.get(key, [&] {
         const long long M = (long long)d.B * d.H * d.W;
         const std::vector<double> dcost = dgrad_block_costs(d);
@@ -516,7 +630,9 @@
             double planes = (double)w.ksplit * w.taps * d.ngroups;
             if (w.plan) { planes = 0.0; for (int i = 0; i < d.ngroups * 9; i++) planes += (double)w.plan[2 * i]; }
             const double tail = 3.0 + 2.4 * planes * ((double)cout * cin / (512.0 * 4608.0));
-            MergedGroupsPlan p = merged_groups_decide(dcost, wgrad_block_costs(w), cus);
+            const std::vector<double> wcost = wgrad_block_costs(w);
+            MergedGroupsPlan p = merged_groups_decide_orders(dcost, wgrad_block_costs(wgrad_shape_on(w, xcd_loads(dcost), cus)), wcost,
+                                                             dgrad_block_costs(dgrad_shape_on(d, xcd_loads(wcost))), cus);
             p.merged_us += tail;
             p.separate_us += tail;
             p.ksplit = w.plan ? 0 : w.ksplit;
@@ -541,5 +657,19 @@
         return best;
     });
 }
-
-}
+struct MergedHalves { DgradShape d; WgradShape w; };
+inline const MergedHalves &merged_groups_halves(const DgradShape &d, int cin, int cout, int k, const IgemmVariant &v, int ksplit, int w_first, int cus) {
+    static PlanMemo<std::array<int, 23>, MergedHalves> memo;
+    const int vbits = v.skip_dead_steps | v.class_tiles_allowed << 1 | v.class_tiles_forced << 2 | v.wgrad_work_list << 3 | v.wgrad_compact << 4 |
+                      v.xcd_balance << 5;
+    const std::array<int, 23> key = {d.ngroups, d.B, d.H, d.W, cin, cout, k, d.dil[0], d.dil[1], d.dil[2], d.dil[3], d.tiles_m, d.xcd_mix,
+                                     d.row_tiles, d.cls_tiles, d.skip_taps, d.grid, vbits, ksplit, cus, d.balance, d.xrows, w_first};
+    return memo.get(key, [&] {
+        MergedHalves h{d, wgrad_shape_for(d.ngroups, d.B, d.H, d.W, cin, cout, k, d.dil, v, ksplit, cus)};
+        if (w_first) h.d = dgrad_shape_on(d, xcd_loads(wgrad_block_costs(h.w)));
+        else h.w = wgrad_shape_on(h.w, xcd_loads(dgrad_block_costs(d)), cus);
+        return h;
+    });
+}
+
+}
diff --git a/dsrg_amd/ops.py b/dsrg_amd/ops.py
--- a/dsrg_amd/ops.py
+++ b/dsrg_amd/ops.py
@@ -996,7 +996,7 @@
     return p.dtype == torch.bfloat16 and tuple(p.shape) == (rows, chunk_channels // 64, ksize * ksize, 64) and p.is_contiguous()
 
 
-def conv_igemm(xs, packed, biases, dilations, ksize, relu, dropout_p=0.0, seed=0, stream_k=True):
+def conv_igemm(xs, packed, biases, dilations, ksize, relu, dropout_p=0.0, seed=0, stream_k=True, outs=None):
     n = len(xs)
     B, cin, H, W = xs[0].shape
     cout = packed[0].shape[0]
@@ -1007,7 +1007,9 @@
         raise ValueError("conv_igemm needs bf16 CUDA inputs of one shape and kernels packed by pack_conv_weight")
     xs = [x.contiguous(memory_format=cl) for x in xs]
     bs = [None if b is None else _f32c(b, "bias") for b in (biases or [None] * n)]
-    ys = [torch.empty((B, cout, H, W), dtype=torch.bfloat16, device=xs[0].device, memory_format=cl) for _ in range(n)]
+    ys = [torch.empty((B, cout, H, W), dtype=torch.bfloat16, device=xs[0].device, memory_format=cl) for _ in range(n)] if outs is None else list(outs)
+    if not (len(ys) == n and all(_is_bf16(y, (B, cout, H, W), True) for y in ys)):
+        raise ValueError("conv_igemm: outs must be bf16 channels_last tensors of the output's shape")
     ws = _igemm_sk_workspace(xs[0].device) if stream_k else None
     check(_lib.lib().dsrg_conv_igemm_bf16(_ptrs(xs), _ptrs(packed), _ptrs(bs), _ptrs(ys), _i32s(dilations), n, B, H, W, cin, cout, ksize,
                                           int(bool(relu)), float(dropout_p), int(seed) & 0xFFFFFFFFFFFFFFFF, _ptr(ws),
@@ -1054,7 +1056,7 @@
     return gp
 
 
-def conv_igemm_dgrad(gs, packed_t, masks, dilations, ksize, mask_scale=1.0, bias_grad=True, gb_outs=None):
+def conv_igemm_dgrad(gs, packed_t, masks, dilations, ksize, mask_scale=1.0, bias_grad=True, gb_outs=None, gx_outs=None):
     n = len(gs)
     B, cin, H, W = gs[0].shape
     cout = packed_t[0].shape[0]
@@ -1065,7 +1067,9 @@
                for g, p, m in zip(gs, packed_t, masks)):
         raise ValueError("conv_igemm_dgrad needs bf16 channels_last gradients / masks of one shape and packed kernels")
     gs = [g.contiguous(memory_format=cl) for g in gs]
-    outs = [torch.empty((B, cout, H, W), dtype=torch.bfloat16, device=gs[0].device, memory_format=cl) for _ in range(n)]
+    outs = [torch.empty((B, cout, H, W), dtype=torch.bfloat16, device=gs[0].device, memory_format=cl) for _ in range(n)] if gx_outs is None else list(gx_outs)
+    if not (len(outs) == n and all(_is_bf16(o, (B, cout, H, W), True) for o in outs)):
+        raise ValueError("conv_igemm_dgrad: gx_outs must be bf16 channels_last tensors of the data gradient's shape")
     L = _lib.lib()
     gb = ws = None
     if bias_grad:
```
